# vadimkantorov/convasr

Hardware: AMD Instinct MI355X
Metric: audio-seconds/sec/node (fwd+bwd+CTC) at bs64x15s (higher is better)
Workload: dtype bf16

## Files before the change

convasr_amd/_lib.py:

```python
import ctypes
import os

import torch

_HERE = os.path.dirname(os.path.abspath(__file__))
LIB_PATH = os.environ.get('CONVASR_HIP_LIB') or os.path.join(_HERE, 'libconvasr_hip.so')

F32, BF16, I16, F16 = 0, 1, 2, 3
LOSS_SCALER_FLOATS = 8
ACT_NONE, ACT_RELU, ACT_HARDTANH, ACT_LEAKY_RELU = 0, 1, 2, 3
PACK_FWD, PACK_DGRAD = 0, 1
W_REFERENCE, W_KMAJOR = 0, 1
METRIC_CHARS, METRIC_WORDS = 0, 1
METRIC_MAX_LEN = 16383

c_int, c_i64, c_u64, c_f32, c_p = ctypes.c_int, ctypes.c_int64, ctypes.c_uint64, ctypes.c_float, ctypes.c_void_p

_SIGNATURES = dict(
	convasr_abi_version = (c_int, []),
	convasr_last_error = (ctypes.c_char_p, []),
	convasr_convert_layout = (c_int, [c_p, c_int, c_i64, c_i64, c_i64, c_p, c_int, c_i64, c_i64, c_i64, c_int, c_int, c_int, c_p]),
	convasr_signal_absmax = (c_int, [c_p, c_int, c_int, c_int, c_p, c_p]),
	convasr_logmel_fwd = (c_int, [c_p, c_int, c_p, c_p, c_p, c_int, c_p, c_p, c_p, c_int, c_int, c_int, c_int, c_int, c_f32, c_p]),
	convasr_instnorm_fwd = (c_int, [c_p, c_int, c_i64, c_i64, c_i64, c_p, c_int, c_i64, c_i64, c_i64, c_p, c_int, c_int, c_int, c_int, c_f32, c_p]),
	convasr_instnorm_running_fwd = (c_int, [c_p, c_int, c_i64, c_i64, c_i64, c_p, c_int, c_i64, c_i64, c_i64, c_int, c_int, c_int, c_int, c_f32, c_p, c_p, c_p, c_f32, c_int, c_p, c_p]),
	convasr_output_lengths = (c_int, [c_p, c_int, c_int, c_p, c_p]),
	convasr_conv_cout_pad = (c_int, [c_int]),
	convasr_pack_conv_weight = (c_int, [c_p, c_p, c_p, c_int, c_int, c_int, c_int, c_int, c_p]),
	convasr_fold2_geometry = (c_int, [c_int, c_int, ctypes.POINTER(c_int), ctypes.POINTER(c_int)]),
	convasr_fold2_pack_weight = (c_int, [c_p, c_int, c_p, c_int, c_int, c_int, c_int, c_int, c_p]),
	convasr_fold2_unfold_wgrad = (c_int, [c_p, c_p, c_int, c_int, c_int, c_int, c_int, c_int, c_p]),
	convasr_conv1d_fwd = (c_int, [c_p, c_p, c_p, c_int, c_int, c_int, c_int, c_int, c_int, c_int, c_int, c_int, c_int, c_int, c_p, c_p, c_p, c_p, c_int, c_f32, c_f32, c_p, c_p, c_p]),
	convasr_conv_stats_max_rows = (c_int, [c_int, c_int]),
	convasr_grouped_conv1d_fwd = (c_int, [c_p, c_p, c_i64, c_i64, c_i64, c_p, c_p, c_int, c_int, c_int, c_int, c_int, c_int, c_int, c_int, c_int, c_int, c_int, c_p]),
	convasr_grouped_conv1d_dgrad = (c_int, [c_p, c_p, c_p, c_i64, c_i64, c_i64, c_p, c_int, c_int, c_int, c_int, c_int, c_int, c_int, c_int, c_int, c_int, c_p]),
	convasr_grouped_conv1d_wgrad_workspace_bytes = (c_i64, [c_int, c_int, c_int, c_int, c_int]),
	convasr_grouped_conv1d_wgrad = (c_int, [c_p, c_p, c_p, c_p, c_i64, c_i64, c_i64, c_p, c_p, c_int, c_int, c_int, c_int, c_int, c_int, c_int, c_int, c_int, c_int, c_int, c_p]),
	convasr_reduce_rows = (c_int, [c_p, c_int, c_int, c_p, c_p]),
	convasr_debug_set_conv_v2 = (c_int, [c_int]),
	convasr_conv1d_wgrad_workspace_bytes = (c_i64, [c_int, c_int, c_int, c_int, c_int, c_int, c_int, c_int]),
	convasr_conv1d_wgrad = (c_int, [c_p, c_p, c_p, c_p, c_p, c_int, c_int, c_int, c_int, c_int, c_int, c_int, c_int, c_int, c_int, c_int, c_int, c_p]),
	convasr_bn_finalize = (c_int, [c_p, c_int, c_i64, c_p, c_p, c_p, c_p, c_f32, c_f32, c_p, c_p, c_p, c_p, c_int, c_p, c_p]),
	convasr_bn_eval_scale_shift = (c_int, [c_p, c_p, c_p, c_p, c_f32, c_p, c_p, c_int, c_p]),
	convasr_bn_act_fwd = (c_int, [c_p, c_p, c_int, c_p, c_p, c_int, c_p, c_p, c_p, c_int, c_f32, c_f32, c_f32, c_u64, c_u64, c_p, c_p, c_int, c_int, c_int, c_p, c_p]),
	convasr_bn_bwd_workspace_bytes = (c_i64, [c_int, c_int, c_int]),
	convasr_bn_act_bwd_reduce = (c_int, [c_p, c_p, c_p, c_int, c_p, c_p, c_p, c_p, c_int, c_p, c_p, c_p, c_p, c_p, c_p, c_int, c_f32, c_f32, c_f32, c_u64, c_u64, c_p, c_p, c_p, c_p, c_p, c_p, c_p, c_p, c_int, c_int, c_int, c_int, c_p, c_p]),
	convasr_bn_act_bwd_apply = (c_int, [c_p, c_p, c_p, c_int, c_p, c_int, c_p, c_p, c_int, c_f32, c_f32, c_f32, c_u64, c_u64, c_p, c_p, c_int, c_int, c_int, c_p, c_p]),
	convasr_bn_bwd_apply = (c_int, [c_p, c_p, c_p, c_int, c_p, c_p, c_p, c_p, c_p, c_p, c_int, c_int, c_int, c_int, c_p]),
	convasr_log_softmax_fwd = (c_int, [c_p, c_p, c_i64, c_int, c_p]),
	convasr_log_softmax_bwd = (c_int, [c_p, c_p, c_p, c_i64, c_int, c_p]),
	convasr_ctc_workspace_bytes = (c_i64, [c_int, c_int, c_int]),
	convasr_ctc_loss = (c_int, [c_p, c_p, c_p, c_p, c_p, c_p, c_p, c_int, c_int, c_int, c_int, c_int, c_p]),
	convasr_scale_rows = (c_int, [c_p, c_p, c_p, c_i64, c_p, c_int, c_i64, c_p]),
	convasr_loss_head = (c_int, [c_p, c_p, c_i64, c_p, c_int, c_f32, c_p, c_p, c_p, c_p, c_f32, c_p]),
	convasr_entropy = (c_int, [c_p, c_p, c_p, c_int, c_int, c_int, c_f32, c_p]),
	convasr_weighted_mean_entropy = (c_int, [c_p, c_p, c_p, c_int, c_int, c_int, c_int, c_f32, c_p]),
	convasr_argmax = (c_int, [c_p, c_p, c_i64, c_int, c_p]),
	convasr_sumsq_workspace_bytes = (c_i64, []),
	convasr_sumsq = (c_int, [c_p, c_i64, c_p, c_p, c_p, c_f32, c_p, c_p]),
	convasr_sgd_step = (c_int, [c_p, c_p, c_p, c_p, c_i64, c_p, c_f32, c_f32, c_f32, c_f32, c_int, c_int, c_p, c_f32, c_p, c_int, c_p, c_p, c_p, c_p]),
	convasr_adamw_step = (c_int, [c_p, c_p, c_p, c_p, c_i64, c_p, c_f32, c_f32, c_f32, c_f32, c_f32, c_f32, c_p, c_p, c_p, c_f32, c_p, c_int, c_p, c_p, c_p, c_p]),
	convasr_conv1d_dgrad_bn_reduce = (c_int, [c_p, c_p, c_p, c_int, c_int, c_int, c_int, c_int, c_int, c_int, c_int, c_int, c_p, c_p, c_p, c_p, c_p, c_int, c_f32, c_f32, c_f32, c_u64, c_u64, c_p, c_p, c_p, c_p, c_p, c_p]),
	convasr_bn_bwd_finalize = (c_int, [c_p, c_int, c_p, c_p, c_p, c_p, c_p, c_p, c_int, c_i64, c_int, c_p]),
	convasr_novograd_step = (c_int, [c_p, c_p, c_p, c_p, c_p, c_p, c_p, c_int, c_i64, c_p, c_int, c_p, c_p, c_f32, c_f32, c_f32, c_f32, c_f32, c_f32, c_int, c_int, c_p, c_p, c_f32, c_p, c_int, c_p, c_p, c_p, c_p]),
	convasr_step_begin = (c_int, [c_p, c_p]),
	convasr_conv1x1_grouped = (c_int, [c_int, c_p, c_p, c_p, c_p, c_p, c_p, c_p, c_p, c_int, c_int, c_int, ctypes.POINTER(c_int), c_p]),
	convasr_add16 = (c_int, [c_p, c_p, c_p, c_i64, c_int, c_p]),
	convasr_bn_bwd_reduce_many_workspace_bytes = (c_i64, [c_int, c_int, c_int, c_int]),
	convasr_bn_bwd_reduce_many = (c_int, [c_p, c_p, c_f32, c_p, c_int, c_p, c_p, c_p, c_p, c_p, c_p, c_p, c_p, c_p, c_int, c_int, c_int, c_int, c_p]),
	convasr_pack_dgrad_item_bytes = (c_int, []),
	convasr_pack_dgrad_grouped = (c_int, [c_p, c_int, c_int, c_p]),
	convasr_bn_finalize_grouped = (c_int, [c_int, c_p, c_int, c_i64, c_p, c_p, c_p, c_p, c_p, c_p, c_p, c_p, c_int, c_p]),
	convasr_bn_bwd_finalize_grouped = (c_int, [c_int, c_p, c_p, c_p, c_p, c_p, c_p, c_p, c_p, c_p, c_i64, c_int, c_p]),
	convasr_bn_bwd_apply_grouped = (c_int, [c_p, c_int, c_p, c_p, c_p, c_int, c_int, c_int, c_int, c_p]),
	convasr_wgrad1x1_grouped_workspace_bytes = (c_i64, [c_int, c_p, c_p, c_int, c_int]),
	convasr_wgrad1x1_grouped = (c_int, [c_int, c_p, c_p, c_p, c_p, c_p, c_p, c_p, c_p, c_int, c_int, c_int, c_p]),
	convasr_copy = (c_int, [c_p, c_p, c_i64, c_p]),
	convasr_colsum_workspace_bytes = (c_i64, [c_i64, c_int]),
	convasr_colsum = (c_int, [c_p, c_int, c_i64, c_int, c_p, c_p, c_int, c_p]),
	convasr_cast_scale = (c_int, [c_p, c_int, c_p, c_int, c_i64, c_f32, c_p]),
	convasr_bn_act_fwd_split3 = (c_int, [c_p, c_p, c_int, c_p, c_p, c_int, c_p, c_p, c_p, c_int, c_f32, c_f32, c_f32, c_u64, c_u64, c_p, c_p, c_int, c_int, c_int, c_p, c_p]),
	convasr_bn_act_bwd_apply_split3 = (c_int, [c_p, c_p, c_p, c_int, c_p, c_int, c_p, c_p, c_int, c_f32, c_f32, c_f32, c_u64, c_u64, c_p, c_p, c_int, c_int, c_int, c_p, c_p]),
	convasr_split3 = (c_int, [c_p, c_p, c_int, c_i64, c_int, c_int, c_p]),
	convasr_pack_conv_weight_split3 = (c_int, [c_p, c_int, c_p, c_p, c_int, c_int, c_int, c_int, c_int, c_p]),
	convasr_bn_act_bwd_apply_to_half = (c_int, [c_p, c_p, c_p, c_int, c_p, c_int, c_p, c_p, c_int, c_f32, c_f32, c_f32, c_u64, c_u64, c_p, c_p, c_int, c_int, c_int, c_p, c_p]),
	convasr_conv1d_fwd_splitk_plan = (c_int, [c_int, c_int, c_int, c_int, c_int, c_int, c_p]),
	convasr_conv1d_fwd_splitk = (c_int, [c_p, c_p, c_p, c_int, c_int, c_int, c_int, c_int, c_int, c_int, c_int, c_int, c_int, c_p, c_p, c_p, c_int, c_f32, c_f32, c_p, c_int, c_p, c_p]),
	convasr_conv1d_wgrad_ld_supported = (c_int, [c_int] * 10),
	convasr_conv1d_wgrad_ld = (c_int, [c_p, c_int, c_p, c_int, c_p, c_p, c_int, c_int, c_int, c_int, c_int, c_int, c_int, c_int, c_int, c_int, c_int, c_p]),
	convasr_novograd_item_elems = (c_i64, []),
	convasr_collate_pad = (c_int, [c_p, c_p, c_p, c_p, c_int, c_int, c_int, c_i64, c_p]),
	convasr_ctc_alignment_workspace_bytes = (c_i64, [c_int, c_int, c_int]),
	convasr_ctc_alignment = (c_int, [c_p, c_p, c_p, c_p, c_p, c_p, c_int, c_int, c_int, c_int, c_int, c_p]),
	convasr_ctc_alignment_long_states_per_block = (c_int, []),
	convasr_ctc_alignment_long_chunk_frames = (c_int, []),
	convasr_ctc_alignment_long_workspace_bytes = (c_i64, [c_int, c_int, c_int]),
	convasr_ctc_alignment_long = (c_int, [c_p, c_p, c_p, c_p, c_p, c_p, c_i64, c_int, c_int, c_int, c_int, c_int, c_int, c_p]),
	convasr_ctc_alignment_long_parts = (c_int, [c_p, c_p, c_p, c_p, c_p, c_p, c_i64, c_int, c_int, c_int, c_int, c_int, c_int, c_int, c_p]),
	convasr_ctc_beam_search_workspace_bytes = (c_i64, [c_int] * 6),
	convasr_ctc_beam_search = (c_int, [c_p, c_p, c_p, c_p, c_p, c_p, c_p, c_int, c_int, c_int, c_int, c_int, c_int, c_f32, c_int, c_p]),
	convasr_ctc_beam_search_lm_workspace_bytes = (c_i64, [c_int] * 6),
	convasr_ctc_beam_search_lm = (c_int, [c_p, c_p, c_p, c_p, c_p, c_p, c_p, c_int, c_int, c_int, c_int, c_int, c_int, c_f32, c_int,
	                                      c_p, c_p, c_p, c_int, c_p, c_p, c_int, c_p, c_int, c_int, c_int, c_int, ctypes.c_double, ctypes.c_double, c_p]),
	convasr_ctc_beam_search_wide_workspace_bytes = (c_i64, [c_int] * 6),
	convasr_ctc_beam_search_wide = (c_int, [c_p, c_p, c_p, c_p, c_p, c_p, c_p, c_int, c_int, c_int, c_int, c_int, c_int, c_f32, c_int, c_p]),
	convasr_ctc_beam_search_lm_wide_workspace_bytes = (c_i64, [c_int] * 6),
	convasr_ctc_beam_search_lm_wide = (c_int, [c_p, c_p, c_p, c_p, c_p, c_p, c_p, c_int, c_int, c_int, c_int, c_int, c_int, c_f32, c_int,
	                                           c_p, c_p, c_p, c_int, c_p, c_p, c_int, c_p, c_int, c_int, c_int, c_int, ctypes.c_double, ctypes.c_double, c_p]),
	convasr_edit_distance = (c_int, [c_p, c_p, c_p, c_i64, c_p, c_i64, c_p, c_p, c_int, c_int, c_int, c_int, c_int, c_i64, c_p]),
	convasr_ctc_greedy_collapse = (c_int, [c_p, c_p, c_p, c_p, c_int, c_int, c_int, c_int, c_int, c_p]),
	convasr_nw_align_workspace_bytes = (c_i64, [c_int, c_int, c_int]),
	convasr_nw_align = (c_int, [c_p, c_p, c_p, c_p, c_p, c_p, c_p, c_p, c_p, c_i64, c_int, c_int, c_int, c_int, c_int, c_int, c_int, c_p]),
	convasr_sliding_max_out_len = (c_i64, [c_i64, c_int]),
	convasr_sliding_max_tile = (c_int, [c_int]),
	convasr_sliding_max = (c_int, [c_p, c_p, c_int, c_i64, c_int, c_int, c_p]),
	convasr_kth_value_workspace_bytes = (c_i64, [c_int]),
	convasr_kth_value = (c_int, [c_p, c_p, c_p, c_i64, c_int, c_i64, c_i64, c_p]),
	convasr_scan_tile = (c_int, []),
	convasr_sign_prefix_sum_workspace_bytes = (c_i64, [c_i64]),
	convasr_sign_prefix_sum = (c_int, [c_p, c_p, c_p, c_i64, c_i64, c_p]),
	convasr_select_speaker_out_len = (c_i64, [c_i64, c_int, c_int, c_int]),
	convasr_select_speaker_workspace_bytes = (c_i64, [c_i64, c_int, c_int, c_int]),
	convasr_select_speaker = (c_int, [c_p, c_p, c_p, c_p, c_i64, c_i64, c_int, c_int, c_int, c_f32, c_f32, c_f32, c_i64, c_p]),
	convasr_rle1d_workspace_bytes = (c_i64, [c_i64]),
	convasr_rle1d_count_offset = (c_i64, [c_i64]),
	convasr_rle1d_count = (c_int, [c_p, c_int, c_int, c_i64, c_p, c_i64, c_p]),
	convasr_rle1d_write = (c_int, [c_p, c_int, c_int, c_i64, c_p, c_i64, c_i64, c_p, c_p, c_p, c_p]),
	convasr_speaker_error_counts_workspace_bytes = (c_i64, [c_i64]),
	convasr_speaker_error_counts = (c_int, [c_p, c_p, ctypes.POINTER(ctypes.c_int32), c_int, c_i64, c_p, c_p, c_i64, c_p]),
)
SLIDE_ABS, SLIDE_NEG = 1, 2
DIAR_MAX_LEN, DIAR_MAX_KERNEL, RLE_MAX_LEN, SPEAKER_MAX_PERMS = 1 << 28, 16384, 1 << 30, 8

_lib = None


class ConvasrHipError(RuntimeError):
	pass


def declared_symbols():
	return sorted(_SIGNATURES)
# ... 179 lines not shown
```

convasr_amd/csrc/conv.hip:

```cpp
#include "conv_common.h"

template <typename T, bool ALIGNED> __device__ __forceinline__ uint4 load_chunk(const T* row, int e0, int n_valid) {
	constexpr int EPC = 16 / sizeof(T);
	uint4 v = make_uint4(0, 0, 0, 0);
	if (ALIGNED) {
		if (e0 + EPC <= n_valid) v = *reinterpret_cast<const uint4*>(row + e0);
		else if (e0 < n_valid) {
			T tmp[EPC];
#pragma unroll
			for (int i = 0; i < EPC; ++i) tmp[i] = (e0 + i < n_valid) ? row[e0 + i] : (T)0;
			v = *reinterpret_cast<uint4*>(tmp);
		}
	} else if (e0 < n_valid) {
		T tmp[EPC];
#pragma unroll
		for (int i = 0; i < EPC; ++i) tmp[i] = (e0 + i < n_valid) ? row[e0 + i] : (T)0;
		v = *reinterpret_cast<uint4*>(tmp);
	}
	return v;
}

template <typename T, typename O, int XI, bool ALIGNED_X, bool SK = false>
__global__ __launch_bounds__(NTHREADS, sizeof(T) == 4 ? 1 : 2) void conv1d_igemm_kernel(ConvParams p) {
	extern __shared__ __attribute__((aligned(16))) char smem[];
// ... 639 lines not shown
#pragma unroll
				for (int tg_i = 0; tg_i < WG_TG; ++tg_i) {
					if (tg_i < ntaps) {
						uint4 bb[2];
#pragma unroll
						for (int ni = 0; ni < 2; ++ni) {
							const char* bp = xs + ((kk * 16 + kq) * p.stride + tg_i * p.dil) * PITCH + (wn * 64 + ni * 32 + colb) * 2;
							s16x4 lo = __builtin_amdgcn_ds_read_tr16_b64_v4i16((__attribute__((address_space(3))) s16x4*)(bp));
							s16x4 hi = __builtin_amdgcn_ds_read_tr16_b64_v4i16((__attribute__((address_space(3))) s16x4*)(bp + 4 * p.stride * PITCH));
							bb[ni] = make_uint4(__builtin_bit_cast(uint2, lo).x, __builtin_bit_cast(uint2, lo).y, __builtin_bit_cast(uint2, hi).x, __builtin_bit_cast(uint2, hi).y);
						}
#pragma unroll
						for (int mi = 0; mi < 2; ++mi)
#pragma unroll
							for (int ni = 0; ni < 2; ++ni) Mma<T>::run(a[mi], bb[ni], acc[tg_i][mi][ni]);
					}
				}
			}
		} else {
			const int r = lane & 31, h = lane >> 5;
#pragma unroll 4
			for (int k2 = 0; k2 < BKT / 2; ++k2) {
				float a[2];
#pragma unroll
				for (int mi = 0; mi < 2; ++mi) a[mi] = *reinterpret_cast<const float*>(ys + (k2 * 2 + h) * PITCH + (wm * 64 + mi * 32 + r) * 4);
#pragma unroll
				for (int tg_i = 0; tg_i < WG_TG; ++tg_i) {
					if (tg_i < ntaps) {
						float bb[2];
#pragma unroll
						for (int ni = 0; ni < 2; ++ni) bb[ni] = *reinterpret_cast<const float*>(xs + ((k2 * 2 + h) * p.stride + tg_i * p.dil) * PITCH + (wn * 64 + ni * 32 + r) * 4);
#pragma unroll
						for (int mi = 0; mi < 2; ++mi)
#pragma unroll
							for (int ni = 0; ni < 2; ++ni) acc[tg_i][mi][ni] = __builtin_amdgcn_mfma_f32_32x32x2f32(a[mi], bb[ni], acc[tg_i][mi][ni], 0, 0, 0);
					}
				}
			}
		}
		if (c + 1 < c_end) store_tiles(buf ^ 1);
		__syncthreads();
	}

	const int r = lane & 31, h = lane >> 5;
#pragma unroll
	for (int tg_i = 0; tg_i < WG_TG; ++tg_i) {
		if (tg_i < ntaps) {
			float* sl = p.slab + ((int64_t)split * p.K + tap0 + tg_i) * p.Cout * p.Cin;
#pragma unroll
			for (int mi = 0; mi < 2; ++mi)
#pragma unroll
				for (int ni = 0; ni < 2; ++ni) {
					const int ci = ci0 + wn * 64 + ni * 32 + r;
#pragma unroll
					for (int g = 0; g < 16; ++g) {
						const int co = co0 + wm * 64 + mi * 32 + (g & 3) + 8 * (g >> 2) + 4 * h;
						if (co < p.Cout && ci < p.Cin) sl[(int64_t)co * p.Cin + ci] = acc[tg_i][mi][ni][g];
					}
				}
		}
	}
}

__global__ __launch_bounds__(256) void wgrad_reduce_kernel(const float* __restrict__ slab, float* __restrict__ dw, int S, int K, int Cout, int Cin, int accumulate) {
	extern __shared__ float rbuf[];
	const int co = blockIdx.y, ci0 = blockIdx.x * 64;
	const int c = threadIdx.x & 63;
	const int64_t plane = (int64_t)Cout * Cin;
	for (int k = threadIdx.x >> 6; k < K; k += 4) {
		float a = 0.f;
		if (ci0 + c < Cin)
			for (int s = 0; s < S; ++s) a += slab[((int64_t)s * K + k) * plane + (int64_t)co * Cin + ci0 + c];
		rbuf[k * 65 + c] = a;
	}
	__syncthreads();
	const int ncols = min(64, Cin - ci0);
	float* out = dw + ((int64_t)co * Cin + ci0) * K;
	for (int o = threadIdx.x; o < ncols * K; o += 256) {
		const float val = rbuf[(o % K) * 65 + o / K];
		out[o] = accumulate ? out[o] + val : val;
	}
}

__global__ __launch_bounds__(256) void wgrad_reduce_kmajor_kernel(const float* __restrict__ slab, float* __restrict__ dw, int S, int64_t n4, int accumulate) {
	const float4* const s4 = reinterpret_cast<const float4*>(slab);
	float4* const d4 = reinterpret_cast<float4*>(dw);
	for (int64_t i = (int64_t)blockIdx.x * 256 + threadIdx.x; i < n4; i += (int64_t)gridDim.x * 256) {
		float4 a = s4[i];
		for (int s = 1; s < S; ++s) { const float4 b = s4[(int64_t)s * n4 + i]; a.x += b.x; a.y += b.y; a.z += b.z; a.w += b.w; }
		if (accumulate) { const float4 o = d4[i]; a.x += o.x; a.y += o.y; a.z += o.z; a.w += o.w; }
		d4[i] = a;
	}
}

template <typename T> __global__ __launch_bounds__(256) void colsum_kernel(const T* __restrict__ y, float* __restrict__ part, int64_t rows, int C, int rows_per_block) {
	__shared__ float red[4][64];
	const int c = blockIdx.x * 64 + (threadIdx.x & 63), w = threadIdx.x >> 6;
	const int64_t r0 = (int64_t)blockIdx.y * rows_per_block, r1 = min(rows, r0 + rows_per_block);
	float a = 0.f;
	if (c < C)
		for (int64_t rr = r0 + w; rr < r1; rr += 4) a += Elem<T>::load(y + rr * C + c);
	red[w][threadIdx.x & 63] = a;
	__syncthreads();
	if (w == 0 && c < C) part[(int64_t)blockIdx.y * C + c] = red[0][threadIdx.x] + red[1][threadIdx.x] + red[2][threadIdx.x] + red[3][threadIdx.x];
}
__global__ __launch_bounds__(1024) void colsum_final_kernel(const float* __restrict__ part, int nparts, int C, float* __restrict__ out, int accumulate) {
	__shared__ double red[16][64];
	const int cl = threadIdx.x & 63, c = blockIdx.x * 64 + cl, w = threadIdx.x >> 6;
	double a = 0;
	if (c < C)
		for (int i = w; i < nparts; i += 16) a += (double)part[(int64_t)i * C + c];
	red[w][cl] = a;
	__syncthreads();
	if (w != 0 || c >= C) return;
	double s = 0;
	for (int i = 0; i < 16; ++i) s += red[i][cl];
	out[c] = accumulate ? out[c] + (float)s : (float)s;
}

extern "C" int64_t convasr_colsum_workspace_bytes(int64_t rows, int C) { return ceil_div64(rows, 256) * (int64_t)C * 4; }
extern "C" int convasr_colsum(const void* y, int dtype, int64_t rows, int C, float* out, void* workspace, int accumulate, void* stream) {
	CONVASR_CHECK_ARG(y && out && workspace && rows > 0 && C > 0 && (dtype == CONVASR_F32 || convasr_is_half(dtype)), "colsum: bad arguments");
	hipStream_t s = (hipStream_t)stream;
	const int rows_per_block = 256;
	dim3 grid((C + 63) / 64, (unsigned)ceil_div64(rows, rows_per_block));
	float* part = (float*)workspace;
	if (dtype == CONVASR_F32) hipLaunchKernelGGL((colsum_kernel<float>), grid, dim3(256), 0, s, (const float*)y, part, rows, C, rows_per_block);
	else if (dtype == CONVASR_F16) hipLaunchKernelGGL((colsum_kernel<f16_t>), grid, dim3(256), 0, s, (const f16_t*)y, part, rows, C, rows_per_block);
	else hipLaunchKernelGGL((colsum_kernel<bf16_t>), grid, dim3(256), 0, s, (const bf16_t*)y, part, rows, C, rows_per_block);
	hipLaunchKernelGGL(colsum_final_kernel, dim3((C + 63) / 64), dim3(1024), 0, s, (const float*)part, (int)grid.y, C, out, accumulate);
	CONVASR_CHECK_LAUNCH("colsum");
	return 0;
}

extern "C" int64_t convasr_conv1d_wgrad_workspace_bytes(int B, int Cin, int Cout, int Tin, int Tout, int K, int stride, int dil) {
	WgradParams p;
	p.debug = 0;
	p.B = B; p.Cin = Cin; p.Cout = Cout; p.Tin = Tin; p.Tout = Tout; p.K = K; p.stride = stride; p.dil = dil;
	p.pad = 0;
	int splits = 1;
	const int bkt[3] = {64, WgTile<bf16_t>::BKT, WgTile<float>::BKT};
	const double us[3] = {1.6, 2.7, 11.0};
	for (int i = 0; i < 3; ++i) {
		WgradParams q = p;
		wgrad_plan(q, bkt[i], us[i]);
		if (q.splits > splits) splits = q.splits;
	}
	const int64_t slabs = (int64_t)splits * K * (int64_t)Cout * Cin * 4;
	const int64_t dbias_parts = ceil_div64((int64_t)B * Tout, 256) * Cout * 4;
	return slabs > dbias_parts ? slabs : dbias_parts;
}

template <typename T, int XI, bool AX, bool AY> static void launch_wgrad(const WgradParams& p, size_t smem, hipStream_t s) {
	auto kern = conv1d_wgrad_kernel<T, XI, AX, AY>;
	static unsigned long long attr_set = 0;
	convasr_allow_160k_lds(reinterpret_cast<const void*>(kern), attr_set);
	hipLaunchKernelGGL(kern, dim3(p.units * p.splits), dim3(NTHREADS), smem, s, p);
}

template <typename T> static int dispatch_wgrad(WgradParams& p, hipStream_t s) {
	wgrad_plan(p, WgTile<T>::BKT, sizeof(T) == 2 ? 2.7 : 11.0);
	const int xi = (p.x_rows * WgTile<T>::CPR + NTHREADS - 1) / NTHREADS;
	const size_t smem = 2 * (size_t)(WgTile<T>::BKT + p.x_rows) * WgTile<T>::PITCH;
	if (smem > 160 * 1024 || xi > 12) return convasr_fail(CONVASR_EUNSUPPORTED, "conv1d_wgrad: tile too large (x_rows %d)", p.x_rows);
	const bool ax = ((p.Cin * sizeof(T)) & 15) == 0, ay = ((p.Cout * sizeof(T)) & 15) == 0;
	if (ax && ay) { if (xi <= 5) launch_wgrad<T, 5, true, true>(p, smem, s); else launch_wgrad<T, 12, true, true>(p, smem, s); }
	else if (ax) launch_wgrad<T, 12, true, false>(p, smem, s);
	else if (ay) launch_wgrad<T, 12, false, true>(p, smem, s);
	else launch_wgrad<T, 12, false, false>(p, smem, s);
	return 0;
}

static int wgrad_impl(const void* x, int x_ld, const void* dy, int dy_ld, float* dw, float* dbias, void* workspace, int dtype, int B, int Cin, int Cout, int Tin,
                      int Tout, int K, int stride, int dil, int pad, int accumulate, int dw_layout, void* stream) {
	CONVASR_CHECK_ARG(x && dy && dw && workspace && B > 0 && Cin > 0 && Cout > 0 && Tin > 0 && Tout > 0 && K > 0 && stride > 0 && dil > 0 && (dw_layout == CONVASR_W_REFERENCE || dw_layout == CONVASR_W_KMAJOR), "conv1d_wgrad: bad arguments");
	CONVASR_CHECK_ARG(dw_layout == CONVASR_W_REFERENCE || (((int64_t)Cout * Cin) & 3) == 0, "conv1d_wgrad: K-major dw needs Cout * Cin %% 4 == 0");
	CONVASR_CHECK_ARG(K <= 64, "conv1d_wgrad: K %d > 64", K);
	WgradParams p;
	p.debug = g_conv_debug;
	p.x = x; p.dy = dy; p.slab = (float*)workspace;
	p.B = B; p.Cin = Cin; p.Cout = Cout; p.Tin = Tin; p.Tout = Tout; p.K = K; p.stride = stride; p.dil = dil; p.pad = pad;
	p.x_ld = x_ld == Cin ? 0 : x_ld; p.dy_ld = dy_ld == Cout ? 0 : dy_ld;
	hipStream_t s = (hipStream_t)stream;
	int rc;
	if (convasr_is_half(dtype) && g_conv_use_v2 && convasr_wgrad_v2_try(p, dtype, s)) rc = 0;
	else if (p.x_ld || p.dy_ld) return convasr_fail(CONVASR_EUNSUPPORTED, "conv1d_wgrad_ld: frames %d / %d elements apart need the LDS-DMA kernel's envelope (16-bit storage, stride 1, Cin %% 128 == 0, Cout %% 128 == 0)", x_ld, dy_ld);
	else if (dtype == CONVASR_F32) rc = dispatch_wgrad<float>(p, s);
	else if (dtype == CONVASR_BF16) rc = dispatch_wgrad<bf16_t>(p, s);
	else if (dtype == CONVASR_F16) rc = dispatch_wgrad<f16_t>(p, s);
	else return convasr_fail(CONVASR_EUNSUPPORTED, "conv1d_wgrad: dtype %d", dtype);
	if (rc) return rc;
	CONVASR_CHECK_LAUNCH("conv1d_wgrad");
	if (dw_layout == CONVASR_W_KMAJOR) {
		const int64_t n4 = (int64_t)K * Cout * Cin / 4;
		int64_t blocks = ceil_div64(n4, 256);
		if (blocks > 2048) blocks = 2048;
		hipLaunchKernelGGL(wgrad_reduce_kmajor_kernel, dim3((unsigned)blocks), dim3(256), 0, s, (const float*)p.slab, dw, p.splits, n4, accumulate);
	} else hipLaunchKernelGGL(wgrad_reduce_kernel, dim3((Cin + 63) / 64, Cout), dim3(256), (size_t)K * 65 * sizeof(float), s, p.slab, dw, p.splits, K, Cout, Cin, accumulate);
	CONVASR_CHECK_LAUNCH("conv1d_wgrad_reduce");
	if (dbias) {
		const int64_t rows = (int64_t)B * Tout;
		const int rows_per_block = 256;
		dim3 grid((Cout + 63) / 64, (unsigned)ceil_div64(rows, rows_per_block));
		float* part = p.slab;
		if (dtype == CONVASR_F32) hipLaunchKernelGGL((colsum_kernel<float>), grid, dim3(256), 0, s, (const float*)dy, part, rows, Cout, rows_per_block);
		else if (dtype == CONVASR_F16) hipLaunchKernelGGL((colsum_kernel<f16_t>), grid, dim3(256), 0, s, (const f16_t*)dy, part, rows, Cout, rows_per_block);
		else hipLaunchKernelGGL((colsum_kernel<bf16_t>), grid, dim3(256), 0, s, (const bf16_t*)dy, part, rows, Cout, rows_per_block);
		hipLaunchKernelGGL(colsum_final_kernel, dim3((Cout + 63) / 64), dim3(1024), 0, s, (const float*)part, (int)grid.y, Cout, dbias, accumulate);
		CONVASR_CHECK_LAUNCH("conv1d_dbias");
	}
	return 0;
}

extern "C" int convasr_conv1d_wgrad(const void* x, const void* dy, float* dw, float* dbias, void* workspace, int dtype, int B, int Cin, int Cout, int Tin,
                                    int Tout, int K, int stride, int dil, int pad, int accumulate, int dw_layout, void* stream) {
	return wgrad_impl(x, 0, dy, 0, dw, dbias, workspace, dtype, B, Cin, Cout, Tin, Tout, K, stride, dil, pad, accumulate, dw_layout, stream);
}

extern "C" int convasr_conv1d_wgrad_ld(const void* x, int x_ld, const void* dy, int dy_ld, float* dw, void* workspace, int dtype, int B, int Cin, int Cout, int Tin,
                                       int Tout, int K, int dil, int pad, int accumulate, int dw_layout, void* stream) {
	CONVASR_CHECK_ARG(x_ld >= Cin && dy_ld >= Cout && (x_ld & 7) == 0 && (dy_ld & 7) == 0 && convasr_is_half(dtype), "conv1d_wgrad_ld: x_ld >= Cin, dy_ld >= Cout, multiples of 8, 16-bit storage");
	return wgrad_impl(x, x_ld, dy, dy_ld, dw, nullptr, workspace, dtype, B, Cin, Cout, Tin, Tout, K, 1, dil, pad, accumulate, dw_layout, stream);
}

extern "C" int convasr_conv1d_wgrad_ld_supported(int dtype, int B, int Cin, int Cout, int Tin, int Tout, int K, int dil, int x_ld, int dy_ld) {
	if (!convasr_is_half(dtype) || B <= 0 || Cin <= 0 || Cout <= 0 || Tin <= 0 || Tout <= 0 || K <= 0 || K > 64 || dil <= 0 || x_ld < Cin || dy_ld < Cout) return 0;
	WgradParams p = WgradParams();
	p.B = B; p.Cin = Cin; p.Cout = Cout; p.Tin = Tin; p.Tout = Tout; p.K = K; p.stride = 1; p.dil = dil;
	p.x_ld = x_ld == Cin ? 0 : x_ld; p.dy_ld = dy_ld == Cout ? 0 : dy_ld;
	return g_conv_use_v2 && convasr_wgrad_v2_supports(p);
}

static bool fold2_geometry(int K, int pad, int* Kf, int* Pf, int* s0) {
	if (K < 1 || pad < 0) return false;
	*Pf = (pad + 1) / 2;
	*s0 = 2 * *Pf - pad;
	*Kf = (K - 1 + *s0) / 2 + 1;
	return true;
}

extern "C" int convasr_fold2_geometry(int K, int pad, int* K_folded, int* pad_folded) {
	int s0;
	CONVASR_CHECK_ARG(K_folded && pad_folded && fold2_geometry(K, pad, K_folded, pad_folded, &s0), "fold2_geometry: bad arguments");
	return 0;
}

template <typename T>
__global__ __launch_bounds__(256) void fold2_pack_kernel(const float* __restrict__ w, int kmajor, T* __restrict__ wf, int Cout, int CoutPad, int Cin, int K, int Kf, int s0) {
	const int64_t n = (int64_t)Kf * CoutPad * 2 * Cin;
	for (int64_t i = (int64_t)blockIdx.x * 256 + threadIdx.x; i < n; i += (int64_t)gridDim.x * 256) {
		const int c2 = (int)(i % (2 * Cin));
		const int64_t r = i / (2 * Cin);
		const int co = (int)(r % CoutPad), j = (int)(r / CoutPad);
		const int p = c2 >= Cin ? 1 : 0, ci = c2 - p * Cin, k = 2 * j + p - s0;
		float v = 0.f;
		if (co < Cout && k >= 0 && k < K) v = kmajor ? w[((int64_t)k * Cout + co) * Cin + ci] : w[((int64_t)co * Cin + ci) * K + k];
		Elem<T>::store(wf + i, v);
	}
}

extern "C" int convasr_fold2_pack_weight(const float* w, int w_layout, void* packed_fwd, int dtype, int Cout, int Cin, int K, int pad, void* stream) {
	int Kf, Pf, s0;
	CONVASR_CHECK_ARG(w && packed_fwd && Cout > 0 && Cin > 0 && fold2_geometry(K, pad, &Kf, &Pf, &s0) && (w_layout == CONVASR_W_REFERENCE || w_layout == CONVASR_W_KMAJOR), "fold2_pack_weight: bad arguments");
	const int co_pad = convasr_conv_cout_pad(Cout);
	int64_t blocks = ceil_div64((int64_t)Kf * co_pad * 2 * Cin, 256);
	if (blocks > 2048) blocks = 2048;
	if (dtype == CONVASR_BF16) hipLaunchKernelGGL((fold2_pack_kernel<bf16_t>), dim3((unsigned)blocks), dim3(256), 0, (hipStream_t)stream, w, w_layout == CONVASR_W_KMAJOR, (bf16_t*)packed_fwd, Cout, co_pad, Cin, K, Kf, s0);
	else if (dtype == CONVASR_F16) hipLaunchKernelGGL((fold2_pack_kernel<f16_t>), dim3((unsigned)blocks), dim3(256), 0, (hipStream_t)stream, w, w_layout == CONVASR_W_KMAJOR, (f16_t*)packed_fwd, Cout, co_pad, Cin, K, Kf, s0);
	else if (dtype == CONVASR_F32) hipLaunchKernelGGL((fold2_pack_kernel<float>), dim3((unsigned)blocks), dim3(256), 0, (hipStream_t)stream, w, w_layout == CONVASR_W_KMAJOR, (float*)packed_fwd, Cout, co_pad, Cin, K, Kf, s0);
	else return convasr_fail(CONVASR_EUNSUPPORTED, "fold2_pack_weight: dtype %d", dtype);
	CONVASR_CHECK_LAUNCH("fold2_pack_weight");
	return 0;
}

__global__ __launch_bounds__(256) void fold2_unfold_kernel(const float* __restrict__ dwf, float* __restrict__ dw, int kmajor, int Cout, int Cin, int K, int s0, int accumulate) {
	const int64_t n = (int64_t)K * Cout * Cin;
	for (int64_t i = (int64_t)blockIdx.x * 256 + threadIdx.x; i < n; i += (int64_t)gridDim.x * 256) {
		int k, co, ci;
		if (kmajor) { ci = (int)(i % Cin); const int64_t r = i / Cin; co = (int)(r % Cout); k = (int)(r / Cout); }
		else { k = (int)(i % K); const int64_t r = i / K; ci = (int)(r % Cin); co = (int)(r / Cin); }
		const int j = (k + s0) >> 1, p = (k + s0) & 1;
		const float v = dwf[((int64_t)j * Cout + co) * 2 * Cin + p * Cin + ci];
		dw[i] = accumulate ? dw[i] + v : v;
	}
}

extern "C" int convasr_fold2_unfold_wgrad(const float* dw_folded, float* dw, int dw_layout, int Cout, int Cin, int K, int pad, int accumulate, void* stream) {
	int Kf, Pf, s0;
	CONVASR_CHECK_ARG(dw_folded && dw && Cout > 0 && Cin > 0 && fold2_geometry(K, pad, &Kf, &Pf, &s0) && (dw_layout == CONVASR_W_REFERENCE || dw_layout == CONVASR_W_KMAJOR), "fold2_unfold_wgrad: bad arguments");
	int64_t blocks = ceil_div64((int64_t)K * Cout * Cin, 256);
	if (blocks > 2048) blocks = 2048;
	hipLaunchKernelGGL(fold2_unfold_kernel, dim3((unsigned)blocks), dim3(256), 0, (hipStream_t)stream, dw_folded, dw, dw_layout == CONVASR_W_KMAJOR, Cout, Cin, K, s0, accumulate);
	CONVASR_CHECK_LAUNCH("fold2_unfold_wgrad");
	return 0;
}
```

convasr_amd/csrc/misc.hip:

```cpp
#include "common.h"

thread_local char g_convasr_err[512] = {0};

int convasr_fail(int code, const char* fmt, ...) {
	va_list ap;
	va_start(ap, fmt);
	vsnprintf(g_convasr_err, sizeof(g_convasr_err), fmt, ap);
	va_end(ap);
	return code;
}

extern "C" int convasr_abi_version(void) { return CONVASR_ABI_VERSION; }
extern "C" const char* convasr_last_error(void) { return g_convasr_err; }

template <typename S, typename D>
__global__ __launch_bounds__(256) void convert_layout_kernel(const S* __restrict__ src, int64_t ssb, int64_t ssc, int64_t sst,
                                                             D* __restrict__ dst, int64_t dsb, int64_t dsc, int64_t dst_st, int C, int T) {
	__shared__ float tile[64][65];
	const int b = blockIdx.z, c0 = blockIdx.y * 64, t0 = blockIdx.x * 64;
	const int tx = threadIdx.x & 63, ty = threadIdx.x >> 6;
	const bool src_t_fast = (sst == 1) || (ssc != 1), dst_t_fast = (dst_st == 1) || (dsc != 1);
#pragma unroll 4
	for (int i = 0; i < 16; ++i) {
		int c = src_t_fast ? c0 + ty + 4 * i : c0 + tx, t = src_t_fast ? t0 + tx : t0 + ty + 4 * i;
// ... 339 lines not shown
}

extern "C" int convasr_cast_scale(const void* src, int src_dtype, void* dst, int dst_dtype, int64_t n, float scale, void* stream) {
	CONVASR_CHECK_ARG(src && dst && n > 0 && (n & 7) == 0 && ((src_dtype == CONVASR_F32 && convasr_is_half(dst_dtype)) || (convasr_is_half(src_dtype) && dst_dtype == CONVASR_F32)), "cast_scale: n %% 8 == 0, fp32 -> bf16 / fp16 or back");
	int64_t blocks = ceil_div64(n >> 3, 256);
	if (blocks > 8192) blocks = 8192;
	const dim3 g((unsigned)blocks), b(256);
	hipStream_t s = (hipStream_t)stream;
	if (src_dtype == CONVASR_F32) CONVASR_DISPATCH_HALF(dst_dtype, H, hipLaunchKernelGGL((cast_scale_kernel<float, H>), g, b, 0, s, (const float*)src, (H*)dst, n >> 3, scale));
	else CONVASR_DISPATCH_HALF(src_dtype, H, hipLaunchKernelGGL((cast_scale_kernel<H, float>), g, b, 0, s, (const H*)src, (float*)dst, n >> 3, scale));
	CONVASR_CHECK_LAUNCH("cast_scale");
	return 0;
}

__global__ __launch_bounds__(256) void copy_kernel(const unsigned char* __restrict__ src, unsigned char* __restrict__ dst, int64_t n16, int64_t nbytes, int aligned) {
	const int64_t i0 = (int64_t)blockIdx.x * 256 + threadIdx.x, step = (int64_t)gridDim.x * 256;
	if (aligned) {
		for (int64_t i = i0; i < n16; i += step) reinterpret_cast<uint4*>(dst)[i] = reinterpret_cast<const uint4*>(src)[i];
		for (int64_t i = n16 * 16 + i0; i < nbytes; i += step) dst[i] = src[i];
	} else {
		for (int64_t i = i0; i < nbytes; i += step) dst[i] = src[i];
	}
}

extern "C" int convasr_copy(const void* src, void* dst, int64_t nbytes, void* stream) {
	CONVASR_CHECK_ARG(src && dst && nbytes >= 0, "copy: bad arguments");
	if (nbytes == 0) return 0;
	const int aligned = ((((uintptr_t)src) | ((uintptr_t)dst)) & 15) == 0;
	const int64_t n16 = aligned ? nbytes >> 4 : 0;
	int64_t blocks = ceil_div64(aligned ? (n16 > 0 ? n16 : 1) : nbytes, 256);
	if (blocks > 4096) blocks = 4096;
	hipLaunchKernelGGL(copy_kernel, dim3((unsigned)blocks), dim3(256), 0, (hipStream_t)stream, (const unsigned char*)src, (unsigned char*)dst, n16, nbytes, aligned);
	CONVASR_CHECK_LAUNCH("copy");
	return 0;
}

extern "C" int convasr_loss_head(const float* loss_vec, const int64_t* ylen, int64_t ylen_stride, const float* entropy, int B, float accumulate_iterations, float* out3,
                                 float* grad_loss_vec, unsigned char* skipped, const float* loss_scaler, float metric_scale, void* stream) {
	CONVASR_CHECK_ARG(loss_vec && ylen && out3 && B > 0 && accumulate_iterations > 0.f, "loss_head: bad arguments");
	hipLaunchKernelGGL(loss_head_kernel, dim3(1), dim3(256), 0, (hipStream_t)stream, loss_vec, ylen, ylen_stride, entropy, B, accumulate_iterations, out3, grad_loss_vec, skipped, loss_scaler, metric_scale);
	CONVASR_CHECK_LAUNCH("loss_head");
	return 0;
}

#define SUMSQ_BLOCKS 2048
__global__ __launch_bounds__(256) void sumsq_kernel(const float* __restrict__ g, int64_t n, double* __restrict__ part) {
	__shared__ float red[4];
	float acc = 0.f;
	const int64_t n4 = n >> 2;
	const float4* g4 = reinterpret_cast<const float4*>(g);
	for (int64_t i = (int64_t)blockIdx.x * 256 + threadIdx.x; i < n4; i += (int64_t)gridDim.x * 256) {
		float4 v = g4[i];
		acc += v.x * v.x + v.y * v.y + v.z * v.z + v.w * v.w;
	}
	if (blockIdx.x == 0 && threadIdx.x < (n & 3)) { float v = g[n4 * 4 + threadIdx.x]; acc += v * v; }
	acc = wave_sum(acc);
	if ((threadIdx.x & 63) == 0) red[threadIdx.x >> 6] = acc;
	__syncthreads();
	if (threadIdx.x == 0) part[blockIdx.x] = (double)red[0] + (double)red[1] + (double)red[2] + (double)red[3];
}

__global__ __launch_bounds__(256) void sumsq_final_kernel(const double* __restrict__ part, int blocks, double* __restrict__ out, float* __restrict__ norm_out, float norm_scale, const float* __restrict__ scaler) {
	__shared__ double red[256];
	double a = 0;
	for (int i = threadIdx.x; i < blocks; i += 256) a += part[i];
	red[threadIdx.x] = a;
	__syncthreads();
	if (threadIdx.x == 0) { double s = 0; for (int i = 0; i < 256; ++i) s += red[i]; *out = s; if (norm_out) *norm_out = (float)(sqrt(s) * (double)norm_scale) * (scaler ? 1.f / scaler[LS_SCALE] : 1.f); }
}

extern "C" int64_t convasr_sumsq_workspace_bytes(void) { return SUMSQ_BLOCKS * (int64_t)sizeof(double); }

extern "C" int convasr_sumsq(const float* g, int64_t n, double* sumsq, void* workspace, float* norm_out, float norm_scale, const float* loss_scaler, void* stream) {
	CONVASR_CHECK_ARG(g && sumsq && workspace && n > 0, "sumsq: bad arguments");
	CONVASR_CHECK_ARG(((uintptr_t)g & 15) == 0, "sumsq: g must be 16-byte aligned");
	int64_t blocks = ceil_div64(n, 1024);
	if (blocks > SUMSQ_BLOCKS) blocks = SUMSQ_BLOCKS;
	hipLaunchKernelGGL(sumsq_kernel, dim3((unsigned)blocks), dim3(256), 0, (hipStream_t)stream, g, n, (double*)workspace);
	hipLaunchKernelGGL(sumsq_final_kernel, dim3(1), dim3(256), 0, (hipStream_t)stream, (const double*)workspace, (int)blocks, sumsq, norm_out, norm_scale, loss_scaler);
	CONVASR_CHECK_LAUNCH("sumsq");
	return 0;
}

template <typename H> __global__ __launch_bounds__(256) void sgd_step_kernel(float* __restrict__ p, const float* __restrict__ g, float* __restrict__ buf, float* __restrict__ gout,
                                                       int64_t n, const double* __restrict__ sumsq, float max_norm, float lr, float mom, float wd, int nesterov, int first,
                                                       const float* __restrict__ loss_gate, float grad_scale, H* __restrict__ p16, const float* __restrict__ scaler_in, float* __restrict__ scaler_out, const float* __restrict__ lr_dev) {
	if (lr_dev) lr = *lr_dev;
	const bool gated = loss_gate && !(fabsf(*loss_gate) < INFINITY);
	const LossScale ls = loss_scale_read(scaler_in, (scaler_in && sumsq) ? *sumsq : 0.0);
	if (scaler_in && blockIdx.x == 0 && threadIdx.x == 0) loss_scale_advance(scaler_in, scaler_out, ls.overflow, gated);
	if (gated || ls.overflow) return;
	grad_scale *= ls.inv;
	float clip = 1.f;
	if (sumsq && max_norm > 0.f) {
		float total = (float)sqrt(*sumsq) * grad_scale;
		float c = max_norm / (total + 1e-6f);
		clip = c < 1.f ? c : 1.f;
	}
	clip *= grad_scale;
	auto update = [&](float gi, float pv, float& bv, float& gout_v) {
		const float gc = gi * clip;
		gout_v = gc;
		float d = gc + wd * pv;
		if (mom != 0.f) {
			bv = first ? d : mom * bv + d;
			d = nesterov ? d + mom * bv : bv;
		}
		return pv - lr * d;
	};
	const int64_t n4 = n >> 2;
	for (int64_t i = (int64_t)blockIdx.x * 256 + threadIdx.x; i < n4; i += (int64_t)gridDim.x * 256) {
		const float4 g4 = reinterpret_cast<const float4*>(g)[i], p4 = reinterpret_cast<const float4*>(p)[i];
		float4 b4 = make_float4(0.f, 0.f, 0.f, 0.f), o4;
		if (mom != 0.f && !first) b4 = reinterpret_cast<const float4*>(buf)[i];
		float4 r;
		r.x = update(g4.x, p4.x, b4.x, o4.x); r.y = update(g4.y, p4.y, b4.y, o4.y); r.z = update(g4.z, p4.z, b4.z, o4.z); r.w = update(g4.w, p4.w, b4.w, o4.w);
		reinterpret_cast<float4*>(p)[i] = r;
		if (mom != 0.f) reinterpret_cast<float4*>(buf)[i] = b4;
		if (gout) reinterpret_cast<float4*>(gout)[i] = o4;
		if (p16) reinterpret_cast<uint2*>(p16)[i] = make_uint2(pack16<H>(r.x, r.y), pack16<H>(r.z, r.w));
	}
	if (blockIdx.x == 0 && (int64_t)threadIdx.x < (n & 3)) {
		const int64_t i = (n4 << 2) + threadIdx.x;
		float bv = (mom != 0.f && !first) ? buf[i] : 0.f, go;
		const float r = update(g[i], p[i], bv, go);
		p[i] = r;
		if (mom != 0.f) buf[i] = bv;
		if (gout) gout[i] = go;
		if (p16) Elem<H>::store(p16 + i, r);
	}
}

extern "C" int convasr_sgd_step(float* p, const float* g, float* buf, float* grad_out, int64_t n, const double* sumsq, float max_norm, float lr,
                                float momentum, float weight_decay, int nesterov, int first, const float* loss_gate, float grad_scale, void* p16, int p16_dtype,
                                const float* scaler_in, float* scaler_out, const float* lr_dev, void* stream) {
	CONVASR_CHECK_ARG(p && g && n > 0 && (momentum == 0.f || buf), "sgd_step: bad arguments");
	CONVASR_CHECK_ARG(!p16 || convasr_is_half(p16_dtype), "sgd_step: the mirror's dtype must be CONVASR_BF16 or CONVASR_F16");
	CONVASR_CHECK_ARG((scaler_in == nullptr) == (scaler_out == nullptr) && (!scaler_in || (scaler_in != scaler_out && sumsq)), "sgd_step: the loss scaler needs distinct in / out states and the gradient's sum of squares (its overflow check)");
	int64_t blocks = ceil_div64(n, 256);
	if (blocks > 4096) blocks = 4096;
	CONVASR_DISPATCH_HALF(p16_dtype, H, hipLaunchKernelGGL((sgd_step_kernel<H>), dim3((unsigned)blocks), dim3(256), 0, (hipStream_t)stream, p, g, buf, grad_out, n, sumsq, max_norm, lr, momentum, weight_decay, nesterov, first, loss_gate, grad_scale, (H*)p16, scaler_in, scaler_out, lr_dev));
	CONVASR_CHECK_LAUNCH("sgd_step");
	return 0;
}

template <typename H> __global__ __launch_bounds__(256) void adamw_step_kernel(float* __restrict__ p, const float* __restrict__ g, float* __restrict__ m, float* __restrict__ v,
                                                         int64_t n, const double* __restrict__ sumsq, float max_norm, float lr, float beta1, float beta2, float eps, float wd,
                                                         const float* __restrict__ step_in, float* __restrict__ step_out, const float* __restrict__ loss_gate, float grad_scale,
                                                         H* __restrict__ p16, const float* __restrict__ scaler_in, float* __restrict__ scaler_out, const float* __restrict__ lr_dev) {
	if (lr_dev) lr = *lr_dev;
	const bool gated = loss_gate && !(fabsf(*loss_gate) < INFINITY);
	const LossScale ls = loss_scale_read(scaler_in, (scaler_in && sumsq) ? *sumsq : 0.0);
	const float t0 = *step_in;
	if (blockIdx.x == 0 && threadIdx.x == 0) {
		if (scaler_in) loss_scale_advance(scaler_in, scaler_out, ls.overflow, gated);
		*step_out = (gated || ls.overflow) ? t0 : t0 + 1.f;
	}
	if (gated || ls.overflow) return;
	grad_scale *= ls.inv;
	float clip = 1.f;
	if (sumsq && max_norm > 0.f) {
		const float total = (float)sqrt(*sumsq) * grad_scale;
		const float c = max_norm / (total + 1e-6f);
		clip = c < 1.f ? c : 1.f;
	}
	clip *= grad_scale;
// ... 42 lines not shown
```

convasr_amd/functional.py:

```python
import os

import torch

from . import ops, _lib

_pack_cache = {}
_param_epoch = [0]


def bump_param_epoch():
	_param_epoch[0] += 1


def param_version(w):
	return (w._version, w.data_ptr(), _param_epoch[0])


def packed_weight(w, dtype, mode):
	ver = param_version(w)
	ent = _pack_cache.get((id(w), dtype))
	if ent is not None:
		if mode == _lib.PACK_DGRAD:
			if ent['dgr_ver'] == ver:
				return ent['dgr']
# ... 15 lines not shown
			ent['fwd_ver'] = ver if flat._mirror_ver.get(id(w)) == ver else None
			ent['flat'], ent['mirror'] = flat, flat.data16
	if mode == _lib.PACK_FWD and ent['fwd_ver'] == ver:
		return ent['fwd']
	if mode == _lib.PACK_DGRAD and ent['dgr_ver'] == ver:
		return ent['dgr']
	if mode == _lib.PACK_DGRAD:
		ent['fwd'], ent['dgr'] = ops.pack_weight(w, dtype, None, out = (ent['fwd'], ent['dgr']), fwd_is_current = ent['fwd_ver'] == ver)
		ent['fwd_ver'] = ent['dgr_ver'] = ver
	else:
		ent['fwd'] = ops.pack_weight(w, dtype, _lib.PACK_FWD, out = (ent['fwd'], None))
		ent['fwd_ver'] = ver
	if in_place and dtype in ops.HALF_DTYPES:
		arena[0]._mirror_ver[id(w)] = ver
	return ent['fwd'] if mode == _lib.PACK_FWD else ent['dgr']


_structure_epoch = [0]


def invalidate_pack_cache():
	_pack_cache.clear()
	_split_cache.clear()
	_structure_epoch[0] += 1


_split_cache = {}


def force_repack():
	for ent in _pack_cache.values():
		ent['dgr_ver'] = None
		if ent.get('flat') is None:
			ent['fwd_ver'] = None
	for cache in (Fold2._cache, _HeadPad._cache, _split_cache):
		for ent in cache.values():
			ent['ver'] = None


def split_weight(w, dtype, dgrad_planes = 3):
	ver = param_version(w)
	ent = _split_cache.get((id(w), dtype, dgrad_planes))
	if ent is None:
		ent = _split_cache[(id(w), dtype, dgrad_planes)] = dict(w = w, ver = None, fwd = None, dgr = None)
	if ent['ver'] != ver:
		ent['fwd'], ent['dgr'] = ops.pack_weight_split3(w, dtype, out = (ent['fwd'], ent['dgr']), dgrad_planes = dgrad_planes)
		ent['ver'] = ver
	return ent['fwd'], ent['dgr']


_PLANES_ATTR = '_convasr_planes_only'
_PLANES_CACHE_ATTR = '_convasr_planes_cache'
_nan_cells = {}


def _planes_placeholder(z3, B, C, T):
	dev = z3.device
	cell = _nan_cells.get(dev)
	if cell is None:
		cell = _nan_cells[dev] = torch.full((1, ), float('nan'), dtype = torch.float32, device = dev)
	z = cell.as_strided((B, C, T), (0, 0, 0))
	setattr(z, _PLANES_ATTR, z3)
	return z


def _take_planes(x):
	d = getattr(x, '__dict__', None)
	return d.pop(_PLANES_ATTR, None) if d else None


def split_applies(split, dt, spec, Cin, Cout):
	return split is not None and dt == torch.float32 and spec.stride == 1 and Cin % 64 == 0 and Cout % 8 == 0


def structure_epoch():
	return _structure_epoch[0]


PREPACK = os.environ.get('CONVASR_NO_PREPACK') != '1'
GRAPHS_CAPTURED = [False]
_prepack_streams = {}


GROUPED_PACK_MIN = int(os.environ.get('CONVASR_GROUPED_PACK_MIN', 32))
_pack_tables = {}


def _pack_group(stale, dtype, refresh = True):
	group = []
	if dtype in ops.HALF_DTYPES and len(stale) >= GROUPED_PACK_MIN:
		for w in stale:
			ent = _pack_cache.get((id(w), dtype))
			if ent is None or ent['dgr'] is None:
				continue
			fwd = packed_weight(w, dtype, _lib.PACK_FWD) if refresh else ent['fwd']
			Cout, Cin, K = w.shape
			if fwd is not None and Cout % 2 == 0 and Cin % 2 == 0 and fwd.dtype == dtype:
				group.append((w, ent, fwd))
	return group


def _pack_table(group, dtype):
	import struct
	dev = group[0][0].device
	key = tuple((fwd.data_ptr(), ent['dgr'].data_ptr()) for _, ent, fwd in group)
	tab = _pack_tables.get((dev, dtype, key))
	if tab is None:
		if capturing():
			raise _lib.ConvasrHipError('the dgrad pack table changed while a step graph is being captured (GraphedTrainStep prewarms it: functional.prewarm_dgrad_pack)')
		assert _lib.load().convasr_pack_dgrad_item_bytes() == 40
		blob, first = b'', 0
		for w, ent, fwd in group:
			Cout, Cin, K = w.shape
			blob += struct.pack('<QQiiiiii', fwd.data_ptr(), ent['dgr'].data_ptr(), Cout, Cin, K, ops.cout_pad(Cout), ops.cout_pad(Cin), first)
			first += K * ((Cout + 63) // 64) * ((Cin + 63) // 64)
		tab = _pack_tables[(dev, dtype, key)] = dict(key = key, items = torch.frombuffer(bytearray(blob), dtype = torch.uint8).to(dev), blocks = first, n = len(group))
	return tab


def prewarm_dgrad_pack(weights, dtype):
	group = _pack_group([w for w in weights], dtype, refresh = False)
	if group:
		_pack_table(group, dtype)


def _pack_dgrad_many(stale, dtype):
	group = _pack_group(stale, dtype)
	grouped = {id(w) for w, _, _ in group}
	for w in stale:
		if id(w) not in grouped:
			packed_weight(w, dtype, _lib.PACK_DGRAD)
	if not group:
		return
	tab = _pack_table(group, dtype)
	_lib.call('convasr_pack_dgrad_grouped', _lib.ptr(tab['items']), tab['n'], tab['blocks'], _lib.stream_ptr())
	for w, ent, _ in group:
		ent['dgr_ver'] = param_version(w)


def prepack_dgrad_weights(weights, dtype):
	if not weights:
		return
	dev = weights[0].device
	join_prepack(dev)
	stale = []
	for w in weights:
		ent = _pack_cache.get((id(w), dtype))
		if ent is None or ent['dgr'] is None:
			packed_weight(w, dtype, _lib.PACK_DGRAD)
		elif ent['dgr_ver'] != param_version(w):
			stale.append(w)
	if not stale:
		return
	if not PREPACK or GRAPHS_CAPTURED[0]:
		_pack_dgrad_many(stale, dtype)
		return
	st = _prepack_streams.get(dev)
	if st is None:
		st = _prepack_streams[dev] = [torch.cuda.Stream(device = dev), False]
	side, main = st[0], torch.cuda.current_stream(dev)
	_lib.stream_wait(side, main)
	with torch.cuda.stream(side):
		_pack_dgrad_many(stale, dtype)
	st[1] = True


def join_prepack(device):
	st = _prepack_streams.get(device)
	if st is not None and st[1]:
		_lib.stream_wait(torch.cuda.current_stream(device), st[0])
		st[1] = False


CAPTURING = ops._capturing


def capturing():
	return CAPTURING[0]


class _DropoutState:
	seed = 0x5EEDC0DE
	offset = 0
	dev = {}

	@classmethod
	def next(cls, numel):
		off = cls.offset
		cls.offset += (numel + 3) // 4 + 1
		return cls.seed, off

	@classmethod
	def key(cls, device):
		st = cls.dev.get(device)
		return None if st is None else st['state'].data_ptr() + 16

	@classmethod
	def upload(cls, device):
		signed = cls.seed - (1 << 64) if cls.seed >= (1 << 63) else cls.seed
		st = cls.dev.get(device)
		if st is None:
			st = cls.dev[device] = dict(state = torch.zeros(4, dtype = torch.int64, device = device), seed = None)
		st['state'].copy_(torch.tensor([signed, 0, 0, 0], dtype = torch.int64))
		st['seed'] = cls.seed
		return st


def manual_seed(seed):
	_DropoutState.seed = int(seed) & 0xFFFFFFFFFFFFFFFF
	_DropoutState.offset = 0
	for device in list(_DropoutState.dev):
		_DropoutState.upload(device)


def begin_step(device):
	device = torch.device(device)
	st = _DropoutState.dev.get(device)
	if st is None or st['seed'] != _DropoutState.seed:
		if CAPTURING[0]:
			raise _lib.ConvasrHipError('begin_step: the dropout state of this device must exist before a step is captured (run one eager step first)')
		st = _DropoutState.upload(device)
	_lib.call('convasr_step_begin', st['state'].data_ptr(), _lib.stream_ptr())
	_DropoutState.offset = 0


def _deliver(params, compute):
	live = [p is not None and p.requires_grad for p in params]
	if not any(live):
		return [None] * len(params)
	arenas = [getattr(p, '_convasr_grad', None) if ok else None for p, ok in zip(params, live)]
	if all(a is not None for a, ok in zip(arenas, live) if ok):
		fresh = {bool(getattr(p, '_convasr_fresh', True)) for p, ok in zip(params, live) if ok}
		if len(fresh) != 1:
			raise _lib.ConvasrHipError('gradient arenas of one layer are out of step (mixed fresh / accumulated state)')
		compute(arenas, not fresh.pop())
		for p, ok in zip(params, live):
			if ok:
				p._convasr_fresh = False
				hook = getattr(p, '_convasr_ready', None)
				if hook is not None:
					hook(p)
		return [None] * len(params)
	outs = [torch.empty_like(p, dtype = torch.float32, memory_format = torch.contiguous_format) if ok else None for p, ok in zip(params, live)]
	compute(outs, False)
	return outs


def _deliver_many(groups, compute):
	outs, accs, ret, arena_groups = [], [], [], []
	for params in groups:
		live = [p is not None and p.requires_grad for p in params]
		arenas = [getattr(p, '_convasr_grad', None) if ok else None for p, ok in zip(params, live)]
		if any(live) and all(a is not None for a, ok in zip(arenas, live) if ok):
			fresh = {bool(getattr(p, '_convasr_fresh', True)) for p, ok in zip(params, live) if ok}
			if len(fresh) != 1:
				raise _lib.ConvasrHipError('gradient arenas of one layer are out of step (mixed fresh / accumulated state)')
			outs.append(arenas); accs.append(not fresh.pop()); ret.append([None] * len(params)); arena_groups.append((params, live))
		else:
			o = [torch.empty_like(p, dtype = torch.float32, memory_format = torch.contiguous_format) if ok else None for p, ok in zip(params, live)]
			outs.append(o); accs.append(False); ret.append(o)
	compute(outs, accs)
	for params, live in arena_groups:
		for p, ok in zip(params, live):
			if ok:
				p._convasr_fresh = False
				hook = getattr(p, '_convasr_ready', None)
				if hook is not None:
					hook(p)
	return ret


GROUP_RES = os.environ.get('CONVASR_NO_GROUPED_RES') != '1'
_GACC_ATTR = '_convasr_gacc'
RES_WGRAD_SIDE = os.environ.get('CONVASR_NO_RES_WGRAD_SIDE') != '1'
after_long_launch_hooks = {}
_side_streams = {}


def enable_side_stream_wgrad(device, enabled = True):
	device = torch.device(device)
	_side_streams[device] = torch.cuda.Stream(device = device) if enabled else None


def side_stream(device):
	return _side_streams.get(torch.device(device))


SIDE_KEEPALIVE = os.environ.get('CONVASR_NO_SIDE_KEEPALIVE') != '1'
_side_keepalive = {}


def join_side_streams():
	for dev, side in _side_streams.items():
		if side is not None:
			_lib.stream_wait(torch.cuda.current_stream(dev), side)
	_wgrad_pending.clear()
	for held in _side_keepalive.values():
		del held[:]


WGRAD_AFTER_DGRAD = os.environ.get('CONVASR_WGRAD_AFTER_DGRAD', '0') == '1'
_wgrad_pending = {}


def _join_pending_wgrad(dev):
	if _wgrad_pending.pop(dev, False):
		side = _side_streams.get(dev)
		if side is not None:
			torch.cuda.current_stream(dev).wait_stream(side)


def _run_wgrad(dev, tensors, fn):
	side = _side_streams.get(dev)
	if side is None:
		return fn()
	if WGRAD_AFTER_DGRAD:
		_wgrad_pending[dev] = True
	_lib.stream_wait(side, torch.cuda.current_stream(dev))
	with torch.cuda.stream(side):
		out = fn()
	held = _side_keepalive.setdefault(dev, [])
	if SIDE_KEEPALIVE and len(held) < 16384:
		held.extend(tensors)
	else:
		for t in tensors:
			t.record_stream(side)
	return out


SPLIT_FAMILY, SPLIT_WGRAD_FAMILY = 'conv1d_igemm_v2s_kernel<x3>', 'conv1d_wgrad<x3>'


class ConvSpec:

	def __init__(self, K, stride = 1, dilation = 1, padding = 0):
		self.K, self.stride, self.dilation, self.padding = K, stride, dilation, padding


class Fold2:
	_cache = {}
# ... 260 lines not shown
			dz = ops.add16(dz, acc, out = acc)
		link, fused_sums = ctx.bwd_link, None
		if link is not None:
			if link['dz'] is not None and link['dz'].data_ptr() == dz.data_ptr() and link['dz'].shape == dz.shape:
				fused_sums = link['sums']
			link['dz'] = None

		if n_res == 0 and fused_sums is not None:
			coef = torch.empty(3 * Cout, dtype = torch.float32, device = dev)
			finalize = lambda outs, acc: ops.bn_bwd_finalize(fused_sums, gamma, bnp[0], bnp[1], B * Tout, coef = coef, dgamma = outs[0], dbeta = outs[1], accumulate = acc)
			if gamma.requires_grad or beta.requires_grad:
				dgamma, dbeta = _deliver([gamma, beta], finalize)
			else:
				finalize([None, None], False)
				dgamma = dbeta = None
			dy = ops.bn_act_bwd_apply(dz, y, coef, True, bnp[2], bnp[3], act, xlen = xl, dropout_p = p_drop, seed = seed, offset = offset, gate = ctx.gate, step_key = skey, planes = ctx.split, hi_only = hi)
			g = rsum_of = None
		elif n_res == 0:
			coef = torch.empty(3 * Cout, dtype = torch.float32, device = dev)
			reduce = lambda outs, acc: ops.bn_act_bwd_reduce(dz, y, bnp[2], bnp[3], bnp[0], bnp[1], act, xlen = xl, dropout_p = p_drop, seed = seed, offset = offset, write_g = False, gamma = gamma, coef = coef, dgamma = outs[0], dbeta = outs[1], accumulate = acc, gate = ctx.gate, step_key = skey)
			if gamma.requires_grad or beta.requires_grad:
				dgamma, dbeta = _deliver([gamma, beta], reduce)
			else:
				reduce([None, None], False)
				dgamma = dbeta = None
			dy = ops.bn_act_bwd_apply(dz, y, coef, True, bnp[2], bnp[3], act, xlen = xl, dropout_p = p_drop, seed = seed, offset = offset, gate = ctx.gate, step_key = skey, planes = ctx.split, hi_only = hi)
			g = rsum_of = None
		else:
			bn_idx = [r for r in range(n_res) if res_bnp[r] is not None]
			grouped_bn = None
			if ctx.gate is not None and GROUP_RES and dt in ops.HALF_DTYPES and 1 + len(bn_idx) <= 13:
				sets = [(gamma, beta, bnp, y)] + [(ctx.params[3 + 4 * r + 2], ctx.params[3 + 4 * r + 3], res_bnp[r], res_y[r]) for r in bn_idx]
				coefs = torch.empty(len(sets), 3 * Cout, dtype = torch.float32, device = dev)
				holder = {}
				def many(outs, accs):
					holder['g'] = ops.bn_bwd_reduce_many(dz, ctx.gate, p_drop, [t[3] for t in sets], [t[2][0] for t in sets], [t[2][1] for t in sets], [t[0] for t in sets], [coefs[i] for i in range(len(sets))], [o[0] for o in outs], [o[1] for o in outs], accs)
				dgb = _deliver_many([[gm, bt] for gm, bt, _, _ in sets], many)
				g = holder['g']
				dys = ops.bn_bwd_apply_grouped(g, [t[3] for t in sets], [coefs[i] for i in range(len(sets))])
				(dgamma, dbeta), dy = dgb[0], dys[0]
				grouped_bn = {r: (dgb[1 + i][0], dgb[1 + i][1], dys[1 + i]) for i, r in enumerate(bn_idx)}
				rsum_of = None
		if n_res > 0 and grouped_bn is None:
			sums = torch.empty(2 * Cout * (1 + len(bn_idx)), dtype = torch.float64, device = dev)
			rsum_of = {r: sums[2 * Cout * (1 + i):2 * Cout * (2 + i)] for i, r in enumerate(bn_idx)}
			common = dict(xlen = xl, res = res_y, rscale = [None if p is None else p[2] for p in res_bnp], rshift = [None if p is None else p[3] for p in res_bnp], rmean = [None if p is None else p[0] for p in res_bnp], rinvstd = [None if p is None else p[1] for p in res_bnp], dropout_p = p_drop, seed = seed, offset = offset, step_key = skey)
			first = [r for r in bn_idx if r < 2]
			g = ops.bn_act_bwd_reduce(dz, y, bnp[2], bnp[3], bnp[0], bnp[1], act, rsums = [rsum_of.get(r) if r in first else None for r in range(n_res)], sums = sums[:2 * Cout], **common)
			rest = [r for r in bn_idx if r >= 2]
			while rest:
				batch, rest = rest[:2], rest[2:]
				ops.bn_act_bwd_reduce(g, g, None, None, None, None, (_lib.ACT_NONE, 0.0, 0.0), res = [res_y[r] for r in batch], rscale = [None] * len(batch), rshift = [None] * len(batch), rmean = [common['rmean'][r] for r in batch], rinvstd = [common['rinvstd'][r] for r in batch], rsums = [rsum_of[r] for r in batch], write_g = False)
			grouped_bn = GROUP_RES and dt in ops.HALF_DTYPES and len(bn_idx) >= 1 and len(bn_idx) <= 12
			if grouped_bn:
				coefs = torch.empty(1 + len(bn_idx), 3 * Cout, dtype = torch.float32, device = dev)
				sets = [(gamma, beta, bnp, sums[:2 * Cout])] + [(ctx.params[3 + 4 * r + 2], ctx.params[3 + 4 * r + 3], res_bnp[r], rsum_of[r]) for r in bn_idx]
				dgb = _deliver_many([[gm, bt] for gm, bt, _, _ in sets], lambda outs, accs: ops.bn_bwd_finalize_grouped([t[3] for t in sets], [t[0] for t in sets], [t[2][0] for t in sets], [t[2][1] for t in sets], B * Tout,
					[coefs[i] for i in range(len(sets))], [o[0] for o in outs], [o[1] for o in outs], accs))
				dys = ops.bn_bwd_apply_grouped(g, [y] + [res_y[r] for r in bn_idx], [coefs[i] for i in range(len(sets))])
				(dgamma, dbeta), dy = dgb[0], dys[0]
				grouped_bn = {r: (dgb[1 + i][0], dgb[1 + i][1], dys[1 + i]) for i, r in enumerate(bn_idx)}
			else:
				dgamma, dbeta, dy = _bn_backward_from_g(g, y, gamma, beta, bnp, sums[:2 * Cout], B * Tout)

		if n_res == 0:
			grouped_bn = None
		arena_mode = getattr(weight, '_convasr_grad', None) is not None
		if ctx.split is not None and dy.dtype == torch.float32:
			dy = ops.as_cl(dy, ctx.split) if hi else ops.split3(dy, ctx.split, ops.SPLIT_GRAD)
		if hi and ctx.fold is not None:
			wg = lambda: _deliver([weight], lambda outs, acc: Fold2.wgrad_hi(x, dy, weight, spec, ctx.fold[0], ctx.fold[1], outs[0], acc))
		elif hi:
			wg = lambda: _deliver([weight], lambda outs, acc: ops.conv1d_wgrad_hi(x, dy, Cout, spec.K, spec.dilation, spec.padding, outs[0], accumulate = acc))
		elif ctx.split is not None and ctx.fold is not None:
			wg = lambda: _deliver([weight], lambda outs, acc: Fold2.wgrad_split(x, dy, weight, spec, ctx.fold[0], ctx.fold[1], outs[0], acc))
		elif ctx.split is not None:
			xf, dyf = ops.split3_frames(x), ops.split3_frames(dy)
			wg = lambda: _deliver([weight], lambda outs, acc: ops.conv1d_wgrad(xf, dyf, Cout, spec.K, 1, 3 * spec.dilation, 3 * spec.padding, outs[0], accumulate = acc, work = 2.0 * B * Tout * Cout * weight.shape[1] * spec.K, family = SPLIT_WGRAD_FAMILY))
		elif ctx.fold is not None:
			Bx, Cin, Tin = x.shape
			xv = x.as_strided((Bx, 2 * Cin, Tin // 2), (Tin * Cin, 1, 2 * Cin))
			wg = lambda: _deliver([weight], lambda outs, acc: Fold2.wgrad(xv, dy, weight, spec, ctx.fold[0], ctx.fold[1], outs[0], acc))
		else:
			wg = lambda: _deliver([weight], lambda outs, acc: ops.conv1d_wgrad(x, dy, Cout, spec.K, spec.stride, spec.dilation, spec.padding, outs[0], accumulate = acc))
		after = WGRAD_AFTER_DGRAD and arena_mode and _side_streams.get(dev) is not None
		if arena_mode and not after:
			dw, = _run_wgrad(dev, (x, dy), wg)
		dx = None
		if ctx.x_needs_grad:
			if spec.stride != 1:
				raise _lib.ConvasrHipError('conv1d dgrad with stride > 1 is not implemented (only the prologue conv is strided and its input needs no gradient)')
			dx = _dgrad(x, dy, weight, spec, dt, ctx.producer_link, split = ctx.split, hi = hi)
		if after:
			dw, = _run_wgrad(dev, (x, dy), wg)
		if not arena_mode:
			dw, = wg()

		res_grads = [None] * (5 * n_res)
		pending = []
		wg_group = []
		for r in range(n_res):
			rw, rb, rg, rbeta = ctx.params[3 + 4 * r:3 + 4 * r + 4]
			rx = res_x[r]
			need_rx = ctx.needs_input_grad[6 + 5 * r]
			if res_bnp[r] is None:
				res_grads[5 * r] = g if need_rx else None
				continue
			p = res_bnp[r]
			drg, drbeta, dry = grouped_bn[r] if grouped_bn else _bn_backward_from_g(g, res_y[r], rg, rbeta, p, rsum_of[r], B * Tout)
			drx = None
			if ctx.res_split[r]:
				sp, cin_r = cfg['split'], rw.shape[1]
				hi_r = bool(cfg.get('split_hi_bwd'))
				dry3 = ops.as_cl(dry, sp) if hi_r else ops.split3(dry, sp, ops.SPLIT_GRAD)
				if need_rx and hi_r:
					drx = ops.conv1d(dry3, split_weight(rw, sp, 1)[1], cin_r, 1, 1, 1, 0, out_dtype = torch.float32)
				elif need_rx:
					drx = ops.conv1d(dry3, split_weight(rw, sp)[1], cin_r, 1, 1, 1, 0, out_dtype = torch.float32, work = 2.0 * B * Tout * Cout * cin_r, family = SPLIT_FAMILY)

				def res_wgrad3(outs, acc, rx3 = rx, dry3 = dry3, rb = rb, cin_r = cin_r, hi_r = hi_r):
					if hi_r:
						ops.conv1d_wgrad_hi(rx3, dry3, Cout, 1, 1, 0, outs[0], accumulate = acc)
					else:
						ops.conv1d_wgrad(ops.split3_frames(rx3), ops.split3_frames(dry3), Cout, 1, 1, 3, 0, outs[0], accumulate = acc, work = 2.0 * B * Tout * Cout * cin_r, family = SPLIT_WGRAD_FAMILY)
					if outs[1] is not None and not acc and not (outs[1] is getattr(rb, '_convasr_grad', None) and getattr(rb, '_convasr_grad_is_zero', False)):
						outs[1].zero_()
						rb._convasr_grad_is_zero = outs[1] is getattr(rb, '_convasr_grad', None)
				drw, drb = _deliver([rw, rb], res_wgrad3)
				res_grads[5 * r:5 * r + 5] = [drx, drw, drb, drg, drbeta]
				continue
			if need_rx and ctx.res_gacc[r] is not None and rx.shape[1] % 128 == 0 and Cout % 64 == 0:
				pending.append((r, dry))
			elif need_rx:
				join_prepack(dry.device)
				drx = ops.conv1d(dry, packed_weight(rw, dt, _lib.PACK_DGRAD), rx.shape[1], 1, 1, 1, 0)
			arena = getattr(rw, '_convasr_grad', None) is not None and (rb is None or getattr(rb, '_convasr_grad', None) is not None)
			if GROUP_RES and arena and rw.requires_grad and dt in ops.HALF_DTYPES and rx.shape[1] % 128 == 0 and Cout % 128 == 0 and (rb is None or rb.requires_grad):
				wg_group.append((r, rx, dry))
				res_grads[5 * r:5 * r + 5] = [drx, None, None, drg, drbeta]
				continue
			def res_wgrad(outs, acc, rx = rx, dry = dry, rb = rb):
				ops.conv1d_wgrad(rx, dry, Cout, 1, 1, 1, 0, outs[0], accumulate = acc)
				if outs[1] is not None and not acc and not (outs[1] is getattr(rb, '_convasr_grad', None) and getattr(rb, '_convasr_grad_is_zero', False)):
					outs[1].zero_()
					rb._convasr_grad_is_zero = outs[1] is getattr(rb, '_convasr_grad', None)
			if RES_WGRAD_SIDE and arena:
				drw, drb = _run_wgrad(dry.device, (rx, dry), lambda rw = rw, rb = rb, f = res_wgrad: _deliver([rw, rb], f))
			else:
				drw, drb = _deliver([rw, rb], res_wgrad)
			res_grads[5 * r:5 * r + 5] = [drx, drw, drb, drg, drbeta]
		if pending:
			join_prepack(dev)
			accs = [ctx.res_gacc[r] for r, _ in pending]
			fresh = [a['buf'] is None for a in accs]
			for (r, _), a, fr in zip(pending, accs, fresh):
				if fr:
					a['buf'] = ops.empty_cl(B, res_x[r].shape[1], Tout, dt, dev)
			done = ops.conv1x1_grouped([dry for _, dry in pending], [packed_weight(ctx.params[3 + 4 * r], dt, _lib.PACK_DGRAD) for r, _ in pending], [res_x[r].shape[1] for r, _ in pending], outs = [a['buf'] for a in accs], accumulate = [not fr for fr in fresh])
			if done is None:
				raise _lib.ConvasrHipError('grouped input gradient of the residual branches: a shape left the one-tap kernel\'s envelope between forward and backward')
		if wg_group:
			ps = [(ctx.params[3 + 4 * r], ctx.params[3 + 4 * r + 1]) for r, _, _ in wg_group]
			fresh = [bool(getattr(w, '_convasr_fresh', True)) for w, _ in ps]
			if any(b is not None and bool(getattr(b, '_convasr_fresh', True)) != fr for (_, b), fr in zip(ps, fresh)):
				raise _lib.ConvasrHipError('gradient arenas of one residual branch are out of step (mixed fresh / accumulated state)')

			def run():
# ... 85 lines not shown

class ConvBiasFunction(torch.autograd.Function):

	@staticmethod
	def forward(ctx, cfg, x, weight, bias):
		spec, dt = cfg['spec'], cfg['compute_dtype']
		ctx.producer_link = _take_link(x)
		x = ops.as_cl(x, dt)
		Cout, Cin, K = weight.shape
		ctx.split = None
		if cfg.get('split') is not None and dt == torch.float32 and K == 1 and spec.stride == 1 and spec.padding == 0 and Cin % 128 == 0 and Cout <= HEAD_PAD and os.environ.get('CONVASR_NO_HEAD_PAD') != '1':
			ctx.split = cfg['split']
			B, _, T = x.shape
			x = ops.split3(x, ctx.split, ops.SPLIT_INPUT)
			y = ops.conv1d(x, _HeadPad.split_weight(weight, ctx.split, 1 if cfg.get('split_hi_bwd') else 3)[0], Cout, 1, 1, 1, 0, out_dtype = cfg.get('out_dtype', torch.float32), bias = bias, work = 2.0 * B * T * Cout * Cin, family = SPLIT_FAMILY)
		else:
			y = ops.conv1d(x, packed_weight(weight, dt, _lib.PACK_FWD), weight.shape[0], spec.K, spec.stride, spec.dilation, spec.padding, out_dtype = cfg.get('out_dtype', torch.float32), bias = bias)
		ctx.cfg = cfg
		ctx.params = (weight, bias)
		ctx.save_for_backward(x)
		return y

	@staticmethod
	def backward(ctx, dy):
		cfg = ctx.cfg
		spec, dt = cfg['spec'], cfg['compute_dtype']
		weight, bias = ctx.params
		x, = ctx.saved_tensors
		Cout = weight.shape[0]
		if ctx.split is not None:
			Cin = weight.shape[1]
			B, _, T = dy.shape
			dy = ops.as_cl(dy, torch.float32)
			hi = bool(cfg.get('split_hi_bwd'))
			dy3 = _HeadPad.pad_grad(dy, ctx.split) if hi else ops.split3(_HeadPad.pad_grad(dy, torch.float32), ctx.split, ops.SPLIT_GRAD)
			dx = None
			if ctx.needs_input_grad[1] and hi:
				dx = ops.conv1d(dy3, _HeadPad.split_weight(weight, ctx.split, 1)[1], Cin, 1, 1, 1, 0, out_dtype = torch.float32, work = 2.0 * B * T * Cout * Cin)
				_after_long_launch()
			elif ctx.needs_input_grad[1]:
				dx = ops.conv1d(dy3, _HeadPad.split_weight(weight, ctx.split)[1], Cin, 1, 1, 1, 0, out_dtype = torch.float32, work = 2.0 * B * T * Cout * Cin, family = SPLIT_FAMILY)
				_after_long_launch()

			def wgrad3(outs, acc):
				dwp = torch.empty(HEAD_PAD, Cin, 1, dtype = torch.float32, device = dy.device)
				if hi:
					ops.conv1d_wgrad_hi(x, dy3, HEAD_PAD, 1, 1, 0, dwp, work = 2.0 * B * T * Cout * Cin)
				else:
					ops.conv1d_wgrad(ops.split3_frames(x), ops.split3_frames(dy3), HEAD_PAD, 1, 1, 3, 0, dwp, work = 2.0 * B * T * Cout * Cin, family = SPLIT_WGRAD_FAMILY)
				if outs[0] is not None:
					v = dwp[:Cout]
					if acc:
						outs[0].add_(v.view(outs[0].shape))
					else:
						_lib.call('convasr_convert_layout', _lib.ptr(v), _lib.F32, 0, v.stride(0), v.stride(1), _lib.ptr(outs[0]), _lib.F32, 0, outs[0].stride(0), outs[0].stride(1), 1, Cout, Cin, _lib.stream_ptr())
				if outs[1] is not None:
					ops.colsum(dy, outs[1], accumulate = acc)
			dw, db = _deliver([weight, bias], wgrad3)
			return None, dx, dw, db
		if dt in ops.HALF_DTYPES and spec.K == 1 and spec.stride == 1 and spec.padding == 0 and Cout < HEAD_PAD and x.shape[1] % 128 == 0 and os.environ.get('CONVASR_NO_HEAD_PAD') != '1':
			dyp = _HeadPad.pad_grad(dy, dt)
			dx = _dgrad(x, dyp, weight, spec, dt, ctx.producer_link, wd = _HeadPad.dgrad_weight(weight, dt)) if ctx.needs_input_grad[1] else None

			def wgrad(outs, acc):
				dwp = torch.empty(HEAD_PAD, x.shape[1], 1, dtype = torch.float32, device = x.device)
				dbp = torch.empty(HEAD_PAD, dtype = torch.float32, device = x.device) if outs[1] is not None else None
				ops.conv1d_wgrad(x, dyp, HEAD_PAD, 1, 1, 1, 0, dwp, dbias = dbp)
				for o, v in ((outs[0], dwp[:Cout]), (outs[1], None if dbp is None else dbp[:Cout].view(Cout, 1, 1))):
					if o is None:
						continue
					if acc:
						o.add_(v.view(o.shape))
					else:
						ov = o.view(Cout, -1, 1) if o.ndim == 1 else o
						_lib.call('convasr_convert_layout', _lib.ptr(v), _lib.F32, 0, v.stride(0), v.stride(1), _lib.ptr(ov), _lib.F32, 0, ov.stride(0), ov.stride(1), 1, Cout, v.shape[1], _lib.stream_ptr())
			dw, db = _deliver([weight, bias], wgrad)
			return None, dx, dw, db
		dy = ops.as_cl(dy, dt)
		dx = None
		if ctx.needs_input_grad[1]:
			if spec.stride != 1:
				raise _lib.ConvasrHipError('conv1d dgrad with stride > 1 is not implemented')
			dx = _dgrad(x, dy, weight, spec, dt, ctx.producer_link)
		dw, db = _deliver([weight, bias], lambda outs, acc: ops.conv1d_wgrad(x, dy, Cout, spec.K, spec.stride, spec.dilation, spec.padding, outs[0], dbias = outs[1], accumulate = acc))
		return None, dx, dw, db


class GroupedConvReluFunction(torch.autograd.Function):

	@staticmethod
	def forward(ctx, cfg, x, weight, bias):
		spec, dt = cfg['spec'], cfg['compute_dtype']
		_take_link(x)
		x = ops.as_cl(x, dt)
		y = ops.grouped_conv1d(x, weight.detach(), None if bias is None else bias.detach(), cfg['groups'], spec.stride, spec.padding, relu = True)
		ctx.cfg, ctx.params = cfg, (weight, bias)
		ctx.save_for_backward(x, y)
		return y

	@staticmethod
	def backward(ctx, dy):
		cfg = ctx.cfg
		spec, dt, groups = cfg['spec'], cfg['compute_dtype'], cfg['groups']
		weight, bias = ctx.params
		x, y = ctx.saved_tensors
		dy = ops.as_cl(dy, dt)
		dx = ops.grouped_conv1d_dgrad(dy, y, weight.detach(), x.shape[1], x.shape[2], groups, spec.stride, spec.padding) if ctx.needs_input_grad[1] else None
		dw, db = _deliver([weight, bias], lambda outs, acc: ops.grouped_conv1d_wgrad(x, dy, y, outs[0], outs[1], groups, spec.stride, spec.padding, accumulate = acc))
		return None, dx, dw, db


class ConvBnActEvalFunction:

	@staticmethod
	def apply(cfg, x, weight, bias, scale_shift, xlen, res_list):
		spec, dt, act = cfg['spec'], cfg['compute_dtype'], cfg['act']
		x = ops.as_cl(x, dt)
		Cout = weight.shape[0]
		xl = ops.xlen_f32(xlen, x.device) if (cfg['temporal_mask'] and xlen is not None) else None
		scale, shift = (None, None) if scale_shift is None else (scale_shift[0], scale_shift[1])
		fold = Fold2.plan(x, weight, spec, dt, False)
		sk = not torch.is_grad_enabled()
		split = cfg.get('split_eval')
		if fold is not None:
			xv, Kf, Pf, Tout = fold
			conv = lambda **epilogue: ops.conv1d(xv, Fold2.packed_weight(weight, dt, spec.padding), Cout, Kf, 1, 1, Pf, bias = bias, Tout = Tout, work = 2.0 * x.shape[0] * Tout * Cout * x.shape[1] * spec.K, splitk = sk, **epilogue)
		elif split_applies(split, dt, spec, x.shape[1], Cout):
			x3, wp3 = ops.split3(x, split, ops.SPLIT_INPUT), split_weight(weight, split)[0]
			conv = lambda **epilogue: ops.conv1d(x3, wp3, Cout, spec.K, 1, spec.dilation, spec.padding, out_dtype = torch.float32, bias = bias, work = 2.0 * x.shape[0] * ops.conv_out_len(x.shape[2], spec.K, 1, spec.dilation, spec.padding) * Cout * x.shape[1] * spec.K, family = SPLIT_FAMILY, splitk = sk, **epilogue)
		else:
			wp = packed_weight(weight, dt, _lib.PACK_FWD)
			conv = lambda **epilogue: ops.conv1d(x, wp, Cout, spec.K, spec.stride, spec.dilation, spec.padding, bias = bias, splitk = sk, **epilogue)
		p_drop = float(cfg.get('dropout_p', 0.0))
		if not res_list and p_drop == 0:
			return conv(scale = scale, shift = shift, act = act, xlen = xl)
		y = conv()
		res_y, rscale, rshift = [], [], []
		for rx, rw, rb, rss in res_list:
			rx = ops.as_cl(rx, dt)
			if rw is None:
				res_y.append(rx); rscale.append(None); rshift.append(None)
			elif split_applies(split, dt, ConvSpec(1), rx.shape[1], Cout):
				res_y.append(ops.conv1d(ops.split3(rx, split, ops.SPLIT_INPUT), split_weight(rw, split)[0], Cout, 1, 1, 1, 0, out_dtype = torch.float32, bias = rb, work = 2.0 * rx.shape[0] * rx.shape[2] * Cout * rx.shape[1], family = SPLIT_FAMILY, splitk = sk))
				rscale.append(None if rss is None else rss[0]); rshift.append(None if rss is None else rss[1])
			else:
				res_y.append(ops.conv1d(rx, packed_weight(rw, dt, _lib.PACK_FWD), Cout, 1, 1, 1, 0, bias = rb, splitk = sk))
				rscale.append(None if rss is None else rss[0]); rshift.append(None if rss is None else rss[1])
		seed, offset = _DropoutState.next(y.numel()) if p_drop > 0 else (0, 0)
		return ops.bn_act(y, scale, shift, act, xlen = xl, res = res_y, rscale = rscale, rshift = rshift, dropout_p = p_drop, seed = seed, offset = offset, step_key = _DropoutState.key(y.device) if p_drop > 0 else None)


class ConvBnActFrozenStatsFunction(torch.autograd.Function):

	@staticmethod
	def _affine(bn, gamma, beta):
		if bn is None or not isinstance(bn, torch.nn.modules.batchnorm._BatchNorm):
			return None, None, None, None
		ss = ops.bn_eval_scale_shift(gamma, beta, bn.running_mean, bn.running_var, bn.eps)
		return ss[0], ss[1], bn.running_mean.detach().float(), torch.rsqrt(bn.running_var.detach().float() + bn.eps)

	@staticmethod
	def forward(ctx, cfg, x, weight, bias, gamma, beta, xlen, *flat_res):
		spec, dt, act = cfg['spec'], cfg['compute_dtype'], cfg['act']
		ctx.producer_link = _take_link(x)
		x = ops.as_cl(x, dt)
		dev = x.device
		Cout = weight.shape[0]
		xl = ops.xlen_f32(xlen, dev) if (cfg['temporal_mask'] and xlen is not None) else None
		y = ops.conv1d(x, packed_weight(weight, dt, _lib.PACK_FWD), Cout, spec.K, spec.stride, spec.dilation, spec.padding, bias = bias)
		aff = ConvBnActFrozenStatsFunction._affine(cfg['bn'], gamma, beta)
		n_res = len(flat_res) // 5
		res_x, res_y, res_aff = [], [], []
		for r in range(n_res):
			rx, rw, rb, rg, rbeta = flat_res[5 * r:5 * r + 5]
			rx = ops.as_cl(rx, dt)
			res_x.append(rx)
			if rw is None:
				res_y.append(rx); res_aff.append((None, None, None, None))
			else:
				res_y.append(ops.conv1d(rx, packed_weight(rw, dt, _lib.PACK_FWD), Cout, 1, 1, 1, 0, bias = rb))
				res_aff.append(ConvBnActFrozenStatsFunction._affine(cfg['res_bn'][r], rg, rbeta))
		p_drop = cfg['dropout_p']
		seed, offset = _DropoutState.next(y.numel()) if p_drop > 0 else (0, 0)
		skey = _DropoutState.key(dev) if p_drop > 0 else None
		z = ops.bn_act(y, aff[0], aff[1], act, xlen = xl, res = res_y, rscale = [a[0] for a in res_aff], rshift = [a[1] for a in res_aff], dropout_p = p_drop, seed = seed, offset = offset, step_key = skey)
		ctx.cfg, ctx.n_res, ctx.drop = cfg, n_res, (p_drop, seed, offset, skey)
		ctx.params = (weight, bias, gamma, beta) + tuple(flat_res[5 * r + k] for r in range(n_res) for k in range(1, 5))
		ctx.aff, ctx.res_aff = aff, res_aff
		ctx.x_needs_grad = x.requires_grad or ctx.needs_input_grad[1]
		ctx.save_for_backward(x, y, xl, *res_x, *res_y)
		return z

	@staticmethod
	def _coef(scale, C, dev):
		coef = torch.zeros(3 * C, dtype = torch.float32, device = dev)
		coef[:C] = 1.0 if scale is None else scale
		return coef

	@staticmethod
	def backward(ctx, dz):
		cfg, n_res = ctx.cfg, ctx.n_res
		spec, dt, act = cfg['spec'], cfg['compute_dtype'], cfg['act']
		saved = ctx.saved_tensors
		x, y, xl = saved[:3]
		res_x, res_y = list(saved[3:3 + n_res]), list(saved[3 + n_res:3 + 2 * n_res])
		weight, bias, gamma, beta = ctx.params[:4]
		scale, shift, rmean, rinv = ctx.aff
		p_drop, seed, offset, skey = ctx.drop
		B, Cout, Tout = y.shape
		dev = y.device
		dz = ops.as_cl(dz, dt)
		live = lambda p: p is not None and p.requires_grad
		common = dict(xlen = xl, res = res_y, rscale = [a[0] for a in ctx.res_aff], rshift = [a[1] for a in ctx.res_aff], dropout_p = p_drop, seed = seed, offset = offset, step_key = skey)
		dgamma = dbeta = None
		if scale is not None and (live(gamma) or live(beta)):
			sums = torch.empty(2 * Cout, dtype = torch.float64, device = dev)
			scratch = torch.empty(3 * Cout, dtype = torch.float32, device = dev)
			holder = {}
			def reduce(outs, acc):
				holder['g'] = ops.bn_act_bwd_reduce(dz, y, scale, shift, rmean, rinv, act, sums = sums, write_g = True, gamma = gamma, coef = scratch, dgamma = outs[0], dbeta = outs[1], accumulate = acc, **common)
			dgamma, dbeta = _deliver([gamma, beta], reduce)
			g = holder['g']
		else:
			g = ops.bn_act_bwd_reduce(dz, y, scale, shift, None, None, act, write_g = True, **common)
		dy = g if scale is None else ops.bn_act_bwd_apply(g, y, ConvBnActFrozenStatsFunction._coef(scale, Cout, dev), False)
		dw, db = _deliver([weight, bias], lambda outs, acc: ops.conv1d_wgrad(x, dy, Cout, spec.K, spec.stride, spec.dilation, spec.padding, outs[0], dbias = outs[1], accumulate = acc))
		dx = None
		if ctx.x_needs_grad:
			if spec.stride != 1:
				raise _lib.ConvasrHipError('conv1d dgrad with stride > 1 is not implemented (only the prologue conv is strided and its input needs no gradient)')
			dx = _dgrad(x, dy, weight, spec, dt, ctx.producer_link)
		res_grads = []
		for r in range(n_res):
			rw, rb, rg, rbeta = ctx.params[4 + 4 * r:4 + 4 * r + 4]
			need_rx = ctx.needs_input_grad[7 + 5 * r]
			if rw is None:
				res_grads += [g if need_rx else None, None, None, None, None]
				continue
			rscale, rshift, rrm, rri = ctx.res_aff[r]
			drg = drbeta = None
			if rscale is not None and (live(rg) or live(rbeta)):
				rs = torch.empty(2 * Cout, dtype = torch.float64, device = dev)
				ops.bn_act_bwd_reduce(g, g, None, None, None, None, (_lib.ACT_NONE, 0.0, 0.0), res = [res_y[r]], rscale = [None], rshift = [None], rmean = [rrm], rinvstd = [rri], rsums = [rs], write_g = False)
				def put(outs, acc, rs = rs):
					for o, v in ((outs[0], rs[Cout:]), (outs[1], rs[:Cout])):
						if o is not None:
							o.add_(v.float()) if acc else o.copy_(v.float())
				drg, drbeta = _deliver([rg, rbeta], put)
			dry = g if rscale is None else ops.bn_act_bwd_apply(g, res_y[r], ConvBnActFrozenStatsFunction._coef(rscale, Cout, dev), False)
			join_prepack(dev)
			drx = ops.conv1d(dry, packed_weight(rw, dt, _lib.PACK_DGRAD), res_x[r].shape[1], 1, 1, 1, 0) if need_rx else None
			if rb is not None:
				rb._convasr_grad_is_zero = False
			drw, drb = _deliver([rw, rb], lambda outs, acc, rx = res_x[r], dry = dry: ops.conv1d_wgrad(rx, dry, Cout, 1, 1, 1, 0, outs[0], dbias = outs[1], accumulate = acc))
			res_grads += [drx, drw, drb, drg, drbeta]
		return (None, dx, dw, db, dgamma, dbeta, None, *res_grads)


class LogSoftmaxFunction(torch.autograd.Function):

	@staticmethod
	def forward(ctx, logits):
		lp = ops.log_softmax(ops.as_cl(logits, torch.float32))
		ctx.save_for_backward(lp)
		return lp

	@staticmethod
	def backward(ctx, g):
		lp, = ctx.saved_tensors
		return ops.log_softmax_bwd(g, lp)


class CtcLossFunction(torch.autograd.Function):

	@staticmethod
	def forward(ctx, log_probs, targets, olen, ylen, blank, norm = None):
		lp = ops.as_cl(log_probs, torch.float32)
		need = log_probs.requires_grad
		nll, grad = ops.ctc_loss(lp, targets, olen, ylen, blank, need_grad = need)
		ctx.norm = norm
		if need:
			ctx.save_for_backward(grad)
		if norm is None:
			return nll
		if norm.dtype == torch.int64 and norm.ndim == 1 and norm.device == nll.device:
			return ops.scale_rows(nll, None, norm)
		return nll / norm

	@staticmethod
	def backward(ctx, g):
		grad, = ctx.saved_tensors
		return ops.scale_rows(grad, g, ctx.norm), None, None, None, None, None


def ctc_loss(log_probs, targets, olen, ylen, blank, norm = None):
	return CtcLossFunction.apply(log_probs, targets, olen, ylen, blank, norm)
```

convasr_amd/ops.py:

```python
import math
import os

import ctypes

import torch

from . import _lib
from ._lib import call, ptr, stream_ptr, dtype_code, require_cuda

HALF_DTYPES = (torch.bfloat16, torch.float16)

ACT_CODES = dict(none = _lib.ACT_NONE, relu = _lib.ACT_RELU, hardtanh = _lib.ACT_HARDTANH, leaky_relu = _lib.ACT_LEAKY_RELU)


def act_args(nonlinearity):
	if nonlinearity is None:
		return _lib.ACT_NONE, 0.0, 0.0
	name = nonlinearity[0]
	if name == 'relu':
		return _lib.ACT_RELU, 0.0, 0.0
	if name == 'hardtanh':
		return _lib.ACT_HARDTANH, float(nonlinearity[1]), float(nonlinearity[2])
	if name == 'leaky_relu':
		return _lib.ACT_LEAKY_RELU, float(nonlinearity[1]) if len(nonlinearity) > 1 else 0.01, 0.0
# ... 300 lines not shown
	return dw



SPLIT_INPUT, SPLIT_GRAD = 0, 1


def split3(x, dtype, order):
	B, C, T = x.shape
	assert is_cl(x) and x.dtype == torch.float32 and dtype in HALF_DTYPES and C % 8 == 0
	out = empty_cl(B, 3 * C, T, dtype, x.device)
	_lib.timed('hbm:split3_kernel', 0.0, lambda: call('convasr_split3', ptr(x), ptr(out), dtype_code(dtype), B * T, C, int(order), stream_ptr()), nbytes = float(B * T * C * 10))
	return out


def split3_frames(x3):
	B, C3, T = x3.shape
	assert is_cl(x3) and C3 % 3 == 0
	return x3.as_strided((B, C3 // 3, 3 * T), (T * C3, 1, C3 // 3))


def split3_plane(x3, plane = 0):
	B, C3, T = x3.shape
	C = C3 // 3
	assert is_cl(x3) and C3 % 3 == 0
	out = empty_cl(B, C, T, x3.dtype, x3.device)
	out.permute(0, 2, 1).copy_(x3.as_strided((B, T, C), (T * C3, C3, 1), x3.storage_offset() + plane * C))
	return out


def conv1d_wgrad_hi(x3, dy, Cout, K, dil, pad, dw, accumulate = False, work = None, family = None):
	B, C3, Tin = x3.shape
	Cin, Tout = C3 // 3, dy.shape[2]
	layout = weight_layout(dw)
	assert is_cl(x3) and is_cl(dy) and x3.dtype == dy.dtype and x3.dtype in HALF_DTYPES and layout is not None and dw.dtype == torch.float32 and tuple(dw.shape) == (Cout, Cin, K), (dw.shape, dw.stride())
	skey = (x3.dtype, B, Cin, Cout, Tin, Tout, K, dil)
	ok = _wgrad_ld_ok.get(skey)
	if ok is None:
		ok = _wgrad_ld_ok[skey] = bool(_lib.load().convasr_conv1d_wgrad_ld_supported(dtype_code(x3.dtype), B, Cin, Cout, Tin, Tout, K, dil, C3, Cout))
	if not ok:
		return conv1d_wgrad(split3_plane(x3), dy, Cout, K, 1, dil, pad, dw, accumulate = accumulate, work = work, family = family)
	if K == 1 and (Cout * Cin) % 4 == 0:
		layout = _lib.W_KMAJOR
	wkey = (B, Cin, Cout, Tin, Tout, K, 1, dil)
	nbytes = _wgrad_ws_bytes.get(wkey)
	if nbytes is None:
		nbytes = _wgrad_ws_bytes[wkey] = _lib.load().convasr_conv1d_wgrad_workspace_bytes(*wkey)
	ws = workspace(nbytes, x3.device, 'wgrad')
	_lib.timed(family or 'conv1d_wgrad', 2.0 * B * Tout * Cout * Cin * K if work is None else work, lambda: call('convasr_conv1d_wgrad_ld', ptr(x3), C3, ptr(dy), Cout, ptr(dw), ptr(ws), dtype_code(dy.dtype), B, Cin, Cout, Tin, Tout, K, dil, pad, int(accumulate), layout, stream_ptr()))
	return dw


_wgrad_ld_ok = {}


def pack_weight_split3(w, dtype, out = None, want_dgrad = True, dgrad_planes = 3):
	require_cuda(w)
	w = w.detach()
	layout = weight_layout(w) if w.dtype == torch.float32 else None
	if layout is None:
		w, layout = w.float().contiguous(), _lib.W_REFERENCE
	Cout, Cin, K = w.shape
	fwd, dgr = out if out is not None else (None, None)
	if fwd is None:
		fwd = torch.zeros(K, cout_pad(Cout), 3 * Cin, dtype = dtype, device = w.device)
	if dgr is None and want_dgrad:
		dgr = torch.zeros(K, cout_pad(Cin), dgrad_planes * Cout, dtype = dtype, device = w.device)
	assert dgr is None or dgr.shape[2] == dgrad_planes * Cout
	call('convasr_pack_conv_weight_split3', ptr(w), layout, ptr(fwd), ptr(dgr) if want_dgrad else None, dgrad_planes, dtype_code(dtype), Cout, Cin, K, stream_ptr())
	return fwd, (dgr if want_dgrad else None)


def colsum(y, out, accumulate = False):
	B, C, T = y.shape
	assert is_cl(y) and out.dtype == torch.float32 and out.numel() == C and out.is_contiguous()
	ws = workspace(_lib.load().convasr_colsum_workspace_bytes(B * T, C), y.device, 'colsum')
	call('convasr_colsum', ptr(y), dtype_code(y.dtype), B * T, C, ptr(out), ptr(ws), int(accumulate), stream_ptr())
	return out


_wgrad_ws_bytes = {}


def conv1d_wgrad(x, dy, Cout, K, stride, dil, pad, dw, dbias = None, accumulate = False, work = None, family = None):
	B, Cin, Tin = x.shape
	Tout = dy.shape[2]
	layout = weight_layout(dw)
	assert is_cl(x) and is_cl(dy) and x.dtype == dy.dtype and layout is not None and dw.dtype == torch.float32 and tuple(dw.shape) == (Cout, Cin, K), (dw.shape, dw.stride())
	if K == 1 and (Cout * Cin) % 4 == 0:
		layout = _lib.W_KMAJOR
	wkey = (B, Cin, Cout, Tin, Tout, K, stride, dil)
	nbytes = _wgrad_ws_bytes.get(wkey)
	if nbytes is None:
		nbytes = _wgrad_ws_bytes[wkey] = _lib.load().convasr_conv1d_wgrad_workspace_bytes(*wkey)
	ws = workspace(nbytes, x.device, 'wgrad')
	_lib.timed(family or 'conv1d_wgrad', 2.0 * B * Tout * Cout * Cin * K if work is None else work, lambda: call('convasr_conv1d_wgrad', ptr(x), ptr(dy), ptr(dw), ptr(dbias), ptr(ws), dtype_code(x.dtype), B, Cin, Cout, Tin, Tout, K, stride, dil, pad, int(accumulate), layout, stream_ptr()))
	return dw



def grouped_conv1d(x, w, bias, groups, stride = 1, pad = 0, relu = True):
	B, Cin, Tin = x.shape
	Cout, cgi, K = w.shape
	assert is_cl(x) and w.dtype == torch.float32 and cgi * groups == Cin
	Tout = conv_out_len(Tin, K, stride, 1, pad)
	y = empty_cl(B, Cout, Tout, x.dtype, x.device)
	call('convasr_grouped_conv1d_fwd', ptr(x), ptr(w), w.stride(0), w.stride(1), w.stride(2), ptr(bias), ptr(y), dtype_code(x.dtype), B, Cin, Cout, Tin, Tout, K, stride, pad, groups, int(relu), stream_ptr())
	return y


def grouped_conv1d_dgrad(dy, y_act, w, Cin, Tin, groups, stride = 1, pad = 0):
	B, Cout, Tout = dy.shape
	K = w.shape[2]
	assert is_cl(dy) and (y_act is None or (is_cl(y_act) and y_act.dtype == dy.dtype))
	dx = empty_cl(B, Cin, Tin, dy.dtype, dy.device)
	call('convasr_grouped_conv1d_dgrad', ptr(dy), ptr(y_act), ptr(w), w.stride(0), w.stride(1), w.stride(2), ptr(dx), dtype_code(dy.dtype), B, Cin, Cout, Tin, Tout, K, stride, pad, groups, stream_ptr())
	return dx


def grouped_conv1d_wgrad(x, dy, y_act, dw, dbias, groups, stride = 1, pad = 0, accumulate = False):
	B, Cin, Tin = x.shape
	Cout, Tout, K = dy.shape[1], dy.shape[2], dw.shape[2]
	assert is_cl(x) and is_cl(dy) and dw.dtype == torch.float32 and tuple(dw.shape) == (Cout, Cin // groups, K)
	ws = workspace(_lib.load().convasr_grouped_conv1d_wgrad_workspace_bytes(B, Cin, Cout, K, groups), x.device, 'grouped_wgrad')
	call('convasr_grouped_conv1d_wgrad', ptr(x), ptr(dy), ptr(y_act), ptr(dw), dw.stride(0), dw.stride(1), dw.stride(2), ptr(dbias), ptr(ws), dtype_code(x.dtype), B, Cin, Cout, Tin, Tout, K, stride, pad, groups, int(accumulate), stream_ptr())
	return dw



def bn_finalize(stats, n, gamma, beta, running_mean, running_var, momentum, eps, num_batches_tracked = None):
	if isinstance(stats, ConvStats):
		buf, rows, C = stats.buf, stats.rows, stats.C
	else:
		buf, rows, C = stats, 1, stats.numel() // 2
	out = torch.empty(4, C, dtype = torch.float32, device = buf.device)
	o = out.data_ptr()
	call('convasr_bn_finalize', ptr(buf), rows, n, ptr(gamma), ptr(beta), ptr(running_mean), ptr(running_var), float(momentum), float(eps), o, o + 4 * C, o + 8 * C, o + 12 * C, C, ptr(num_batches_tracked), stream_ptr())
	return out


def _float_array(vals):
	return (ctypes.c_float * max(len(vals), 1))(*[float(v) for v in vals])


def bn_finalize_grouped(stats, n, gammas, betas, running_means, running_vars, momenta, epss, num_batches_tracked):
	k, C, rows = len(stats), stats[0].C, stats[0].rows
	assert all(s_.C == C and s_.rows == rows for s_ in stats)
	out = torch.empty(k, 4, C, dtype = torch.float32, device = stats[0].buf.device)
	call('convasr_bn_finalize_grouped', k, _ptr_array([s_.buf for s_ in stats]), rows, n, _ptr_array(gammas), _ptr_array(betas), _ptr_array(running_means), _ptr_array(running_vars),
		_float_array(momenta), _float_array(epss), _ptr_array([out[i] for i in range(k)]), _ptr_array(num_batches_tracked), C, stream_ptr())
	return [out[i] for i in range(k)]


def bn_bwd_finalize_grouped(sums, gammas, means, invstds, n, coefs, dgammas, dbetas, accumulate):
	k, C = len(sums), sums[0].numel() // 2
	call('convasr_bn_bwd_finalize_grouped', k, _ptr_array(sums), _int_array([1] * k), _ptr_array(gammas), _ptr_array(means), _ptr_array(invstds), _ptr_array(coefs), _ptr_array(dgammas), _ptr_array(dbetas),
		_int_array(accumulate), int(n), C, stream_ptr())


def bn_bwd_reduce_many(dz, gate, dropout_p, ys, means, invstds, gammas, coefs, dgammas, dbetas, accumulate):
	B, C, T = dz.shape
	assert is_cl(dz) and dz.dtype in HALF_DTYPES and all(is_cl(y) and y.dtype == dz.dtype and y.shape == dz.shape for y in ys) and gate.dtype == torch.uint8 and gate.numel() * 8 == dz.numel()
	g = empty_cl(B, C, T, dz.dtype, dz.device)
	k = len(ys)
	ws = workspace(_lib.load().convasr_bn_bwd_reduce_many_workspace_bytes(k, B, T, C), dz.device, 'bn_bwd')
	_lib.timed('hbm:bn_act_bwd_reduce_kernel', 0.0, lambda: call('convasr_bn_bwd_reduce_many', ptr(dz), ptr(gate), float(dropout_p), ptr(g), k, _ptr_array(ys), _ptr_array(means), _ptr_array(invstds), _ptr_array(gammas),
		_ptr_array(coefs), _ptr_array(dgammas), _ptr_array(dbetas), _int_array(accumulate), ptr(ws), dtype_code(dz.dtype), B, T, C, stream_ptr()), nbytes = float(B * T * C * dz.element_size() * (2 + k)))
	return g


def bn_bwd_apply_grouped(g, ys, coefs):
	B, C, T = g.shape
	assert is_cl(g) and g.dtype in HALF_DTYPES and all(is_cl(y) and y.dtype == g.dtype and y.shape == g.shape for y in ys)
	dys = [empty_cl(B, C, T, g.dtype, g.device) for _ in ys]
	_lib.timed('hbm:bn_act_bwd_apply_kernel', 0.0, lambda: call('convasr_bn_bwd_apply_grouped', ptr(g), len(ys), _ptr_array(ys), _ptr_array(coefs), _ptr_array(dys), dtype_code(g.dtype), B, T, C, stream_ptr()), nbytes = float(B * T * C * g.element_size() * (1 + 2 * len(ys))))
	return dys


def bn_eval_scale_shift(gamma, beta, running_mean, running_var, eps):
# ... 88 lines not shown
	targets = targets.to(device = dev, dtype = torch.int64).contiguous()
	if targets.ndim == 1:
		targets = targets.view(B, -1)
	olen = olen.to(device = dev, dtype = torch.int64).contiguous()
	ylen = ylen.to(device = dev, dtype = torch.int64).contiguous()
	S_max = targets.shape[1]
	nbytes = _lib.load().convasr_ctc_workspace_bytes(B, T, S_max)
	if nbytes < 0:
		raise _lib.ConvasrHipError(f'ctc_loss: target length {S_max} unsupported')
	ws = workspace(nbytes, dev, 'ctc')
	nll = torch.empty(B, dtype = torch.float32, device = dev)
	grad = empty_cl(B, C, T, torch.float32, dev) if need_grad else None
	call('convasr_ctc_loss', ptr(log_probs), ptr(targets), ptr(olen), ptr(ylen), ptr(nll), ptr(grad), ptr(ws), B, T, C, S_max, blank, stream_ptr())
	return nll, grad


def scale_rows(grad, gscale, gdiv = None):
	B = grad.shape[0]
	out = torch.empty_like(grad)
	assert gdiv is None or (gdiv.dtype == torch.int64 and gdiv.ndim == 1 and gdiv.shape[0] == B and gdiv.device == grad.device)
	call('convasr_scale_rows', ptr(grad), None if gscale is None else ptr(gscale.to(torch.float32).contiguous()), ptr(gdiv), 0 if gdiv is None else gdiv.stride(0), ptr(out), B, grad.numel() // B, stream_ptr())
	return out


def loss_head(loss_vec, ylen_col, ent = None, accumulate_iterations = 1, need_grad = True, loss_scaler = None, metric_scale = 1.0):
	require_cuda(loss_vec)
	B = loss_vec.shape[0]
	lv = loss_vec.detach().to(torch.float32).contiguous()
	assert ylen_col.dtype == torch.int64 and ylen_col.ndim == 1 and ylen_col.shape[0] == B and ylen_col.device == lv.device
	out3 = torch.empty(3, dtype = torch.float32, device = lv.device)
	gvec = torch.empty(B, dtype = torch.float32, device = lv.device) if need_grad else None
	skipped = torch.empty(1, dtype = torch.bool, device = lv.device)
	ent = None if ent is None else ent.detach().to(torch.float32).contiguous()
	call('convasr_loss_head', ptr(lv), ptr(ylen_col), ylen_col.stride(0), ptr(ent), B, float(accumulate_iterations), ptr(out3), ptr(gvec), ptr(skipped), ptr(loss_scaler), float(metric_scale), stream_ptr())
	return out3, gvec, skipped


def entropy(log_probs, olen = None, eps = 1e-9):
	B, C, T = log_probs.shape
	lp = as_cl(log_probs, torch.float32)
	ent = torch.empty(B, dtype = torch.float32, device = lp.device)
	ol = None if olen is None else olen.to(device = lp.device, dtype = torch.int64).contiguous()
	call('convasr_entropy', ptr(lp), ptr(ol), ptr(ent), B, T, C, float(eps), stream_ptr())
	return ent


def weighted_mean_entropy(log_probs, olen = None, eps = 1e-9, eps_id = -1):
	B, C, T = log_probs.shape
	lp = as_cl(log_probs, torch.float32)
	out = torch.empty(B, dtype = torch.float32, device = lp.device)
	ol = None if olen is None else olen.to(device = lp.device, dtype = torch.int64).contiguous()
	call('convasr_weighted_mean_entropy', ptr(lp), ptr(ol), ptr(out), B, T, C, int(eps_id) % C, float(eps), stream_ptr())
	return out


def normalize_signal(signal, eps = 1e-5, denom_multiplier = 1.0):
	require_cuda(signal)
	assert signal.ndim == 2
	if signal.numel() == 0:
		return signal
	signal = signal.contiguous() if signal.dtype in (torch.float32, torch.int16) else signal.float().contiguous()
	B, T = signal.shape
	absmax = torch.empty(B, dtype = torch.float32, device = signal.device)
	call('convasr_signal_absmax', ptr(signal), dtype_code(signal.dtype), B, T, ptr(absmax), stream_ptr())
	x = signal if signal.dtype == torch.float32 else signal.float()
	out = torch.empty_like(x)
	scale = ((absmax + eps) * denom_multiplier).reciprocal()
	call('convasr_scale_rows', ptr(x), ptr(scale), None, 0, ptr(out), B, T, stream_ptr())
	return out


def argmax(log_probs):
	B, C, T = log_probs.shape
	lp = as_cl(log_probs, torch.float32)
	idx = torch.empty(B, T, dtype = torch.int64, device = lp.device)
	call('convasr_argmax', ptr(lp), ptr(idx), B * T, C, stream_ptr())
	return idx



def sumsq(flat_grad, out = None, norm_out = None, norm_scale = 1.0, loss_scaler = None):
	out = out if out is not None else torch.empty(1, dtype = torch.float64, device = flat_grad.device)
	ws = workspace(_lib.load().convasr_sumsq_workspace_bytes(), flat_grad.device, 'sumsq')
	call('convasr_sumsq', ptr(flat_grad), flat_grad.numel(), ptr(out), ptr(ws), ptr(norm_out), float(norm_scale), ptr(loss_scaler), stream_ptr())
	return out


def _scaler_pair(scaler):
	if scaler is None:
		return None, None
	s_in, s_out = scaler
	assert s_in.dtype == s_out.dtype == torch.float32 and s_in.numel() == s_out.numel() == _lib.LOSS_SCALER_FLOATS and s_in.data_ptr() != s_out.data_ptr()
	return s_in, s_out


def sgd_step(p, g, buf, n, sumsq_buf, max_norm, lr, momentum, weight_decay, nesterov, first, grad_out = None, loss_gate = None, grad_scale = 1.0, p16 = None, scaler = None, lr_dev = None):
	assert loss_gate is None or (loss_gate.dtype == torch.float32 and loss_gate.numel() == 1)
	assert p16 is None or (p16.dtype in HALF_DTYPES and p16.numel() == n)
	s_in, s_out = _scaler_pair(scaler)
	call('convasr_sgd_step', ptr(p), ptr(g), ptr(buf), ptr(grad_out), n, ptr(sumsq_buf), float(max_norm), float(lr), float(momentum), float(weight_decay), int(nesterov), int(first), ptr(loss_gate), float(grad_scale), ptr(p16), _lib.BF16 if p16 is None else dtype_code(p16.dtype), ptr(s_in), ptr(s_out), ptr(lr_dev), stream_ptr())


def adamw_step(p, g, exp_avg, exp_avg_sq, n, sumsq_buf, max_norm, lr, beta1, beta2, eps, weight_decay, step_in, step_out, loss_gate = None, grad_scale = 1.0, p16 = None, scaler = None, lr_dev = None):
	assert loss_gate is None or (loss_gate.dtype == torch.float32 and loss_gate.numel() == 1)
	assert p16 is None or (p16.dtype in HALF_DTYPES and p16.numel() == n)
	assert step_in.dtype == step_out.dtype == torch.float32 and step_in.data_ptr() != step_out.data_ptr()
	s_in, s_out = _scaler_pair(scaler)
	call('convasr_adamw_step', ptr(p), ptr(g), ptr(exp_avg), ptr(exp_avg_sq), n, ptr(sumsq_buf), float(max_norm), float(lr), float(beta1), float(beta2), float(eps), float(weight_decay), ptr(step_in), ptr(step_out), ptr(loss_gate), float(grad_scale), ptr(p16), _lib.BF16 if p16 is None else dtype_code(p16.dtype), ptr(s_in), ptr(s_out), ptr(lr_dev), stream_ptr())


def conv1d_dgrad_bn_reduce(dy, packed_dgrad, Cin, K, dil, pad, bn_y, bn_scale, bn_shift, bn_mean, bn_invstd, act, dropout_p, seed, offset, xlen, bn_sums, work = None, gate = None, step_key = None):
	import ctypes
	B, Cout, Tdy = dy.shape
	T = conv_out_len(Tdy, K, 1, dil, pad)
	assert is_cl(dy) and dy.dtype in HALF_DTYPES and is_cl(bn_y) and bn_y.dtype == dy.dtype and tuple(bn_y.shape) == (B, Cin, T) and isinstance(bn_sums, ConvStats) and bn_sums.fits(Cin, B, T, dy.device), (dy.shape, bn_y.shape, Cin, T)
	rows = ctypes.c_int(0)
	dx = empty_cl(B, Cin, T, dy.dtype, dy.device)
	rc = [0]
	def run():
		rc[0] = _lib.call_rc('convasr_conv1d_dgrad_bn_reduce', ptr(dy), ptr(packed_dgrad), ptr(dx), dtype_code(dy.dtype), B, Cout, Cin, Tdy, T, K, dil, pad, ptr(bn_y), ptr(bn_scale), ptr(bn_shift), ptr(bn_mean), ptr(bn_invstd), act[0], act[1], act[2], float(dropout_p), int(seed), int(offset), step_key, ptr(xlen), ptr(bn_sums.buf), ctypes.byref(rows), ptr(gate), stream_ptr())
	family = 'conv1d_igemm_v2s_kernel<bf16>+bn_bwd' if Cout % 64 == 0 else 'conv1d_igemm (other variants)'
	flops, nbytes_ = 2.0 * B * T * Cout * Cin * K if work is None else work, float(B * Tdy * Cout * 2 + K * Cout * Cin * 2 + 2 * B * T * Cin * 2)
	symbol = 'v2s16' if family.startswith('conv1d_igemm_v2s') else None
	if family.startswith('conv1d_igemm_v2s') and memory_bound(flops, nbytes_):
		family = 'hbm:conv1d_igemm_v2s_kernel (memory-bound launches: the 38-class decoder)'
	_lib.timed(family, flops, run, nbytes = nbytes_, symbol = symbol)
	bn_sums.rows = rows.value
	return dx if rc[0] == 0 else None


def bn_bwd_finalize(sums, gamma, mean, invstd, n, coef = None, dgamma = None, dbeta = None, accumulate = False):
	buf, rows, C = (sums.buf, sums.rows, sums.C) if isinstance(sums, ConvStats) else (sums, 1, sums.numel() // 2)
	call('convasr_bn_bwd_finalize', ptr(buf), rows, ptr(gamma), ptr(mean), ptr(invstd), ptr(coef), ptr(dgamma), ptr(dbeta), int(accumulate), int(n), C, stream_ptr())



def novograd_work_table(offsets_host, device):
	item = _lib.load().convasr_novograd_item_elems()
	items, seg_first = [], [0]
	for s_, (lo, hi) in enumerate(zip(offsets_host[:-1], offsets_host[1:])):
		for b in range(lo, max(hi, lo + 1), item):
			items.append((s_, b, min(hi, b + item)))
		seg_first.append(len(items))
	return (torch.tensor(items, dtype = torch.int64, device = device), torch.tensor(seg_first, dtype = torch.int64, device = device), torch.empty(len(items), dtype = torch.float64, device = device))


def novograd_step(p, g, mom, ema_in, ema_out, g2, offsets, n, table, max_norm, lr, beta1, beta2, eps, weight_decay, dampening, first, loss_gate = None, total_norm = None, grad_scale = 1.0, p16 = None, scaler = None, lr_dev = None):
	items, seg_first, item_part = table
	assert offsets.dtype == torch.int64 and ema_in.data_ptr() != ema_out.data_ptr() and g2.dtype == torch.float64
	n_seg = offsets.numel() - 1
	s_in, s_out = _scaler_pair(scaler)
	assert p16 is None or (p16.dtype in HALF_DTYPES and p16.numel() == n)
	assert int(first) >= 0 or (ema_in.numel() == n_seg + 1 and ema_out.numel() == n_seg + 1), 'first = -1 (device-side first-step detection) needs the applied-step counter behind the EMAs'
	call('convasr_novograd_step', ptr(p), ptr(g), ptr(mom), ptr(ema_in), ptr(ema_out), ptr(g2), ptr(offsets), n_seg, n, ptr(items), items.shape[0], ptr(seg_first), ptr(item_part), float(max_norm or 0.0), float(lr), float(beta1), float(beta2), float(eps), float(weight_decay), int(bool(dampening)), int(first), ptr(loss_gate), ptr(total_norm), float(grad_scale), ptr(p16), _lib.BF16 if p16 is None else dtype_code(p16.dtype), ptr(s_in), ptr(s_out), ptr(lr_dev), stream_ptr())


def ctc_alignment(log_probs_btc, targets, input_lengths, target_lengths, blank):
	B, T, C = log_probs_btc.shape
	dev = log_probs_btc.device
	assert log_probs_btc.is_contiguous() and log_probs_btc.dtype == torch.float32
	targets = targets.to(device = dev, dtype = torch.int64).contiguous()
	il = input_lengths.to(device = dev, dtype = torch.int64).contiguous()
	tl = target_lengths.to(device = dev, dtype = torch.int64).contiguous()
	S_max = targets.shape[1]
	out = torch.empty(B, S_max, dtype = torch.int64, device = dev)
	ws = workspace(_lib.load().convasr_ctc_alignment_workspace_bytes(B, T, S_max), dev, 'ctc_alignment')
	call('convasr_ctc_alignment', ptr(log_probs_btc), ptr(targets), ptr(il), ptr(tl), ptr(out), ptr(ws), B, T, C, S_max, int(blank), stream_ptr())
	return out
# ... 307 lines not shown
```

convasr_amd/parallel.py:

```python
import os
import queue
import threading
import weakref

import torch
import torch.distributed as dist
import torch.nn as nn

from .train import FlatParameters


XGMI_LINK_GBS_PER_DIRECTION = 76.8


def predict_exposed_comm(params_numel, offsets, buckets, world, step_ms, link_gbs = XGMI_LINK_GBS_PER_DIRECTION, efficiency = 0.7, latency_us = 40.0, forward_share = 0.33, tail_share = 0.04, bytes_per_element = 4):
	total = float(sum(params_numel))
	bwd_share = 1.0 - forward_share - tail_share
	t_fwd, t_bwd_end = step_ms * forward_share, step_ms * (forward_share + bwd_share)
	rows, t_free = [], 0.0
	for b in sorted(buckets, key = lambda b: -b['lo']):
		above = sum(n for n, o in zip(params_numel, offsets) if o >= b['lo'])
		ready = t_fwd + (t_bwd_end - t_fwd) * above / total
		nbytes = (b['hi'] - b['lo']) * bytes_per_element
		t = 0.0 if world <= 1 else 2.0 * (nbytes / world) / (efficiency * link_gbs * 1e9) * 1e3 + latency_us * 1e-3
		start = max(ready, t_free)
		t_free = start + t
		rows.append(dict(mib = round(nbytes / 2 ** 20, 1), ready_ms = round(ready, 3), start_ms = round(start, 3), comm_ms = round(t, 3), end_ms = round(t_free, 3)))
	return dict(exposed_comm_ms = round(max(0.0, t_free - t_bwd_end), 3), comm_ms_total = round(sum(r['comm_ms'] for r in rows), 3), backward_end_ms = round(t_bwd_end, 3), step_ms = round(step_ms, 3),
		world = world, link_gbs_per_direction = link_gbs, efficiency = efficiency, latency_us = latency_us, bytes_per_element = bytes_per_element, per_bucket = rows,
		predicted_scaling = None if world <= 1 else round(world * step_ms / (step_ms + max(0.0, t_free - t_bwd_end)), 3),
		model = 'direct reduce-scatter + all-gather over one xGMI link per peer; bucket ready times from the backward pass apportioned by parameter counts; serial collectives on the communication stream (convasr_amd.parallel.predict_exposed_comm)')


class DataParallelEngine(nn.Module):
	def __init__(self, module, device = None, bucket_bytes = int(os.environ.get('CONVASR_BUCKET_MIB', 64)) << 20, process_group = None, flat = None, force_collectives = False, first_bucket_bytes = 4 << 20, fold_mean = True, comm_thread = os.environ.get('CONVASR_COMM_THREAD', '0') == '1', measure_exposed_comm = False, grad_comm_dtype = os.environ.get('CONVASR_GRAD_COMM', 'auto')):
		super().__init__()
		self.module = module
		self.group = process_group
		self.world_size = dist.get_world_size(process_group) if dist.is_initialized() else 1
		self.collectives = self.world_size > 1 or (force_collectives and dist.is_initialized())
		self.flat = flat if flat is not None else getattr(module, '_convasr_flat', None) or FlatParameters(module)
		module._convasr_flat = self.flat
		self.buckets = self._make_buckets(bucket_bytes, min(first_bucket_bytes, bucket_bytes))
		self._pending = []
		self._ready = []
		self._jobs = queue.Queue() if (comm_thread and self.collectives and self.flat.data.is_cuda) else None
		self._worker = None
		self._comm_dirty = False
		self._remaining = [len(b['params']) for b in self.buckets]
		self._main_stream = None
		self._comm_stream = None
		self.fold_mean = fold_mean
		self.sync = True
		self.grad_comm_dtype = {None: None, 'f32': None, 'auto': 'auto', 'f16': torch.float16, 'bf16': torch.bfloat16}.get(grad_comm_dtype, grad_comm_dtype)
		self._comm_bufs = {}
		self._mean_in_comm = False
		self._capture_comm = None
		for bi, b in enumerate(self.buckets):
			for p in b['params']:
				p._convasr_ready = self._make_hook(bi)
		self.measure_exposed_comm = measure_exposed_comm
		self.exposed_comm_events = []
		from . import functional as Fn
		ref, key = weakref.ref(self), id(self)
		def hook():
			eng = ref()
			if eng is None:
				Fn.after_long_launch_hooks.pop(key, None)
			else:
				eng.poll()
		Fn.after_long_launch_hooks[key] = hook
		self._hook_key = key
		if self.collectives:
			dist.broadcast(self.flat.data, src = 0, group = self.group)
			for buf in module.buffers():
				dist.broadcast(buf, src = 0, group = self.group)
			from . import functional as Fn
			Fn.bump_param_epoch()

	def close(self):
		from . import functional as Fn
		Fn.after_long_launch_hooks.pop(getattr(self, '_hook_key', None), None)
		worker, self._worker = getattr(self, '_worker', None), None
		if worker is not None and self._jobs is not None:
			self._jobs.put(None)
			worker.join(timeout = 5)

	def destroy_capture_comm(self):
		comm, self._capture_comm = self._capture_comm, None
		if comm is not None:
			comm.destroy()

	def __del__(self):
		try:
			self.close()
		except Exception:
			pass

	def predict(self, world, step_ms, **kw):
		kw.setdefault('bytes_per_element', 2 if self.comm_dtype() is not None else 4)
		return predict_exposed_comm([p.numel() for p in self.flat.params], self.flat.offsets, self.buckets, world, step_ms, **kw)

	def exposed_comm_ms(self):
		ms = [a.elapsed_time(b) for a, b in self.exposed_comm_events]
		return sum(ms) / len(ms) if ms else None

	def _make_buckets(self, bucket_bytes, first_bucket_bytes):
		flat = self.flat
		buckets, cur = [], None
		for p, off in zip(flat.params, flat.offsets):
			end = off + p.numel()
			limit = min(bucket_bytes, first_bucket_bytes << max(len(buckets) - 1, 0))
			if cur is None or (end - cur['lo']) * 4 > limit and cur['params']:
				cur = dict(lo = off, hi = end, params = [])
				buckets.append(cur)
			cur['params'].append(p)
			cur['hi'] = end
		return buckets

	def _make_hook(self, bi):
		def ready(param):
			if not self.sync:
				return
			self._remaining[bi] -= 1
			if self._remaining[bi] == 0:
				self._mark_ready(bi)
		return ready

	def _comm(self, dev):
		if self._comm_stream is None:
			self._comm_stream = torch.cuda.Stream(device = dev)
		return self._comm_stream

	def _mark_ready(self, bi):
		if not self.collectives:
			return
		view = self.flat.grad[self.buckets[bi]['lo']:self.buckets[bi]['hi']]
		if not view.is_cuda:
			self._launch(bi, ())
			return
		from . import functional as Fn
		dev = view.device
		producers = {s.cuda_stream: s for s in (self._main_stream, torch.cuda.current_stream(dev), Fn.side_stream(dev)) if s is not None}
# ... 194 lines not shown
```

convasr_amd/train.py:

```python
import math
import os

import torch

from . import ops, _lib
from . import models as M
from . import functional as Fn


class FlatParameters:
	ALIGN = 64

	def __init__(self, model):
		params = [p for p in model.parameters() if p.requires_grad]
		if not params:
			raise ValueError('model has no trainable parameters')
		dev = params[0].device
		self.params, self.offsets = params, []
		off = 0
		for p in params:
			if p.dtype != torch.float32 or p.device != dev:
				raise ValueError('FlatParameters needs fp32 parameters on one device')
			self.offsets.append(off)
			off += (p.numel() + self.ALIGN - 1) // self.ALIGN * self.ALIGN
		self.numel = off
		self.data = torch.zeros(off, dtype = torch.float32, device = dev)
		self.grad = torch.zeros(off, dtype = torch.float32, device = dev)
		self.data16 = None
		self._mirror_ver = {}
		self._as_param = []
		for p, o in zip(params, self.offsets):
			n = p.numel()
			kmajor = p.ndim == 3 and p.shape[2] > 1 and (p.shape[0] * p.shape[1]) % 8 == 0 and dev.type == 'cuda'
			as_param = (lambda flat, p = p, o = o, n = n: flat[o:o + n].view(p.shape[2], p.shape[0], p.shape[1]).permute(1, 2, 0)) if kmajor else (lambda flat, p = p, o = o, n = n: flat[o:o + n].view(p.shape))
			self._as_param.append(as_param)
			view = as_param(self.data)
			view.copy_(p.data)
			p.data = view
			p._convasr_grad = as_param(self.grad)
			p._convasr_fresh = True
			one_tap = p.ndim == 3 and p.shape[2] == 1 and (p.shape[0] * p.shape[1]) % 8 == 0 and dev.type == 'cuda'
			p._convasr_arena = (self, o) if (kmajor or one_tap) else None
			p.grad = p._convasr_grad
		self._by_id = {id(p): p for p in params}
		self.clip = None
		self.grad_scale = 1.0
		self._sumsq = torch.zeros(1, dtype = torch.float64, device = dev)
		self.loss_scaler = None

	def mirror(self, dtype = torch.bfloat16):
		if self.data16 is None or self.data16.dtype != dtype:
			assert dtype in ops.HALF_DTYPES
			self.data16 = torch.zeros(self.numel, dtype = dtype, device = self.data.device)
			self._mirror_ver = {}
		return self.data16

	def mirror_carried_over(self, run):
		was = {k for k, v in self._mirror_ver.items() if v == Fn.param_version(self._by_id[k])} if self._mirror_ver else set()
		run(self.data16)
		Fn.bump_param_epoch()
		self._mirror_ver = {k: Fn.param_version(self._by_id[k]) for k in was} if self.data16 is not None else {}

	def param_views(self, flat_tensor):
		assert flat_tensor.numel() == self.numel
		return [f(flat_tensor) for f in self._as_param]

	def export_state(self, flat_tensor):
		return [v.contiguous().clone() for v in self.param_views(flat_tensor)]

	def import_state(self, flat_tensor, per_param, what):
		if isinstance(per_param, torch.Tensor):
			raise ValueError(f'{what}: a flat arena-ordered tensor (optimizer state written before format 2) carries no layout tag and cannot be loaded safely: conv segments may be tap-major or reference-ordered')
		views = self.param_views(flat_tensor)
		if len(per_param) != len(views):
			raise ValueError(f'{what}: {len(per_param)} tensors for {len(views)} parameters')
		for v, t in zip(views, per_param):
			if tuple(v.shape) != tuple(t.shape):
				raise ValueError(f'{what}: shape {tuple(t.shape)} does not match parameter shape {tuple(v.shape)}')
			v.copy_(t)

	def zero_grad(self):
		for p in self.params:
			p._convasr_fresh = True
			p.grad = p._convasr_grad
		self.clip = None

	def grads_written_externally(self):
		for p in self.params:
			if getattr(p, '_convasr_grad_is_zero', False):
				p._convasr_grad_is_zero = False

	def finalize_grads(self):
		for p in self.params:
			if p._convasr_fresh:
				p._convasr_grad.zero_()

	def clip_grad_norm_(self, max_norm):
		self.finalize_grads()
		norm = torch.empty(1, dtype = torch.float32, device = self.grad.device)
		ops.sumsq(self.grad, self._sumsq, norm_out = norm, norm_scale = self.grad_scale, loss_scaler = None if self.loss_scaler is None else self.loss_scaler.current)
		self.clip = (self._sumsq, float(max_norm))
		return norm[0]


class LossScaler:

	def __init__(self, device, loss_scale = 'dynamic', init_scale = 2.0 ** 16, scale_factor = 2.0, scale_window = 2000, min_loss_scale = None, max_loss_scale = 2.0 ** 24):
		dynamic = loss_scale in (None, 'dynamic')
		state = [float(init_scale) if dynamic else float(loss_scale), 0.0, 0.0, float(scale_window) if dynamic else 0.0, float(min_loss_scale or 0.0), float(max_loss_scale), float(scale_factor), 0.0]
		assert len(state) == _lib.LOSS_SCALER_FLOATS
		self.state = torch.tensor([state, state], dtype = torch.float32, device = device)
		self.cur = 0
		self.pinned = False

	@property
	def current(self):
		return self.state[self.cur]

	def pair(self):
		return self.state[self.cur], self.state[1 - self.cur]

	def advance(self):
		if Fn.capturing() or self.pinned:
			_lib.call('convasr_copy', _lib.ptr(self.state[1 - self.cur]), _lib.ptr(self.state[self.cur]), 4 * _lib.LOSS_SCALER_FLOATS, _lib.stream_ptr())
		else:
			self.cur = 1 - self.cur

	def loss_scale(self):
		return float(self.current[0])

	def state_dict(self):
		s = self.current.tolist()
		return dict(loss_scale = s[0], unskipped = int(s[1]))

	def load_state_dict(self, sd):
		cur = self.current.clone()
		cur[0], cur[1] = float(sd['loss_scale']), float(sd['unskipped'])
		self.state[self.cur].copy_(cur)


def amp_state_dict(optimizer):
	scaler = getattr(getattr(optimizer, 'flat', None), 'loss_scaler', None)
	return {} if scaler is None else dict(loss_scaler0 = scaler.state_dict())


def amp_load_state_dict(optimizer, sd):
	scaler = getattr(getattr(optimizer, 'flat', None), 'loss_scaler', None)
	if scaler is not None and sd and 'loss_scaler0' in sd:
		scaler.load_state_dict(sd['loss_scaler0'])


class SGD:

	def __init__(self, flat: FlatParameters, lr = 1e-2, momentum = 0.9, weight_decay = 1e-3, nesterov = False, keep_clipped_grads = False):
		self.flat = flat
		self.param_groups = [dict(params = flat.params, lr = lr, momentum = momentum, weight_decay = weight_decay, nesterov = nesterov)]
		self.momentum_buffer = torch.zeros_like(flat.data) if momentum != 0 else None
		self.steps = 0
		self.keep_clipped_grads = keep_clipped_grads
		self.lr_dev = None

	def zero_grad(self, set_to_none = False):
		self.flat.zero_grad()

	def step(self, loss_gate = None):
		g = self.param_groups[0]
		flat = self.flat
		if flat.clip is None:
			flat.finalize_grads()
		sumsq, max_norm = flat.clip if flat.clip is not None else (None, 0.0)
		first, grad_scale = self.steps == 0, flat.grad_scale
		if first and Fn.capturing():
			raise _lib.ConvasrHipError('SGD: the first step (which initialises the momentum buffer) cannot be the one captured into a step graph')
		scaler = flat.loss_scaler
		if scaler is not None and sumsq is None:
			sumsq = ops.sumsq(flat.grad, flat._sumsq)
		flat.mirror_carried_over(lambda p16: ops.sgd_step(flat.data, flat.grad, self.momentum_buffer, flat.numel, sumsq, max_norm, g['lr'], g['momentum'], g['weight_decay'], g['nesterov'], first, grad_out = flat.grad if self.keep_clipped_grads else None, loss_gate = loss_gate, grad_scale = grad_scale, p16 = p16, scaler = None if scaler is None else scaler.pair(), lr_dev = self.lr_dev if Fn.capturing() else None))
		if scaler is not None:
			scaler.advance()
		if self.keep_clipped_grads:
			flat.grads_written_externally()
		self.steps += 1
		flat.clip, flat.grad_scale = None, 1.0
# ... 306 lines not shown
```

include/convasr_hip.h:

```cpp
#ifndef CONVASR_HIP_H
#define CONVASR_HIP_H

#include <stdint.h>

#ifdef __cplusplus
extern "C" {
#endif

#define CONVASR_ABI_VERSION 10

enum { CONVASR_F32 = 0, CONVASR_BF16 = 1, CONVASR_I16 = 2, CONVASR_F16 = 3 };
enum { CONVASR_ACT_NONE = 0, CONVASR_ACT_RELU = 1, CONVASR_ACT_HARDTANH = 2, CONVASR_ACT_LEAKY_RELU = 3 };
enum { CONVASR_OK = 0, CONVASR_EINVAL = -1, CONVASR_ELAUNCH = -2, CONVASR_EUNSUPPORTED = -3 };

int convasr_abi_version(void);
const char* convasr_last_error(void);


int convasr_convert_layout(const void* src, int src_dtype, int64_t src_sb, int64_t src_sc, int64_t src_st,
                           void* dst, int dst_dtype, int64_t dst_sb, int64_t dst_sc, int64_t dst_st,
                           int B, int C, int T, void* stream);


int convasr_signal_absmax(const void* signal, int signal_dtype, int B, int T, float* absmax, void* stream);

int convasr_logmel_fwd(const void* signal, int signal_dtype, const float* absmax, const float* xlen,
                       const float* window, int win_length, const float* mel_weight, const float* mel_bias,
                       float* out, int B, int T, int nfft, int hop, int nmel, float preemphasis, void* stream);


int convasr_instnorm_fwd(const void* x, int x_dtype, int64_t x_sb, int64_t x_sc, int64_t x_st,
                         void* y, int y_dtype, int64_t y_sb, int64_t y_sc, int64_t y_st,
                         const float* xlen, int B, int C, int T, int T_out, float eps, void* stream);

int convasr_instnorm_running_fwd(const void* x, int x_dtype, int64_t x_sb, int64_t x_sc, int64_t x_st,
                                 void* y, int y_dtype, int64_t y_sb, int64_t y_sc, int64_t y_st,
                                 int B, int C, int T, int T_out, float eps, float* running_mean, float* running_var,
                                 int64_t* num_batches_tracked, float momentum, int training, float* stats_workspace, void* stream);


int convasr_output_lengths(const float* xlen, int B, int T, int64_t* out, void* stream);


int convasr_conv_cout_pad(int cout);

#define CONVASR_W_REFERENCE 0
#define CONVASR_W_KMAJOR 1

int convasr_pack_conv_weight(const float* w, void* packed_fwd, void* packed_dgrad, int dtype, int Cout, int Cin, int K, int w_layout, void* stream);

int convasr_conv1d_fwd(const void* x, const void* wp, void* y, int x_dtype, int y_dtype,
                       int B, int Cin, int Cout, int Tin, int Tout, int K, int stride, int dil, int pad,
                       const float* bias, double* stats, const float* scale, const float* shift,
                       int act, float act_lo, float act_hi, const float* xlen, int* stats_rows, void* stream);
int convasr_conv_stats_max_rows(int B, int Tout);

int convasr_conv1d_fwd_splitk_plan(int x_dtype, int B, int Cin, int Cout, int Tout, int K, int64_t* workspace_bytes);
int convasr_conv1d_fwd_splitk(const void* x, const void* wp, void* y, int x_dtype, int y_dtype,
                              int B, int Cin, int Cout, int Tin, int Tout, int K, int dil, int pad,
                              const float* bias, const float* scale, const float* shift, int act, float act_lo, float act_hi,
                              const float* xlen, int splits, void* workspace, void* stream);

int convasr_fold2_geometry(int K, int pad, int* K_folded, int* pad_folded);
int convasr_fold2_pack_weight(const float* w, int w_layout, void* packed_fwd, int dtype, int Cout, int Cin, int K, int pad, void* stream);
int convasr_fold2_unfold_wgrad(const float* dw_folded, float* dw, int dw_layout, int Cout, int Cin, int K, int pad, int accumulate, void* stream);

int convasr_debug_set_conv_v2(int enable);

int64_t convasr_conv1d_wgrad_workspace_bytes(int B, int Cin, int Cout, int Tin, int Tout, int K, int stride, int dil);

int convasr_conv1d_wgrad(const void* x, const void* dy, float* dw, float* dbias, void* workspace, int dtype,
                         int B, int Cin, int Cout, int Tin, int Tout, int K, int stride, int dil, int pad,
                         int accumulate, int dw_layout, void* stream);


int convasr_grouped_conv1d_fwd(const void* x, const float* w, int64_t w_sco, int64_t w_sj, int64_t w_sk, const float* bias, void* y, int dtype,
                               int B, int Cin, int Cout, int Tin, int Tout, int K, int stride, int pad, int groups, int relu, void* stream);
int convasr_grouped_conv1d_dgrad(const void* dy, const void* y_act, const float* w, int64_t w_sco, int64_t w_sj, int64_t w_sk, void* dx, int dtype,
                                 int B, int Cin, int Cout, int Tin, int Tout, int K, int stride, int pad, int groups, void* stream);
int64_t convasr_grouped_conv1d_wgrad_workspace_bytes(int B, int Cin, int Cout, int K, int groups);
int convasr_grouped_conv1d_wgrad(const void* x, const void* dy, const void* y_act, float* dw, int64_t w_sco, int64_t w_sj, int64_t w_sk, float* dbias,
                                 void* workspace, int dtype, int B, int Cin, int Cout, int Tin, int Tout, int K, int stride, int pad, int groups,
                                 int accumulate, void* stream);


int convasr_bn_finalize(const double* stats, int stats_rows, int64_t n, const float* gamma, const float* beta,
                        float* running_mean, float* running_var, float momentum, float eps,
                        float* mean, float* invstd, float* scale, float* shift, int C,
                        int64_t* num_batches_tracked, void* stream);
int convasr_reduce_rows(const double* part, int rows, int width, double* out, void* stream);

int convasr_bn_eval_scale_shift(const float* gamma, const float* beta, const float* running_mean, const float* running_var,
                                float eps, float* scale, float* shift, int C, void* stream);

int convasr_bn_act_fwd(const void* y, void* z, int dtype, const float* scale, const float* shift,
                       int n_res, const void* const* res, const float* const* rscale, const float* const* rshift,
                       int act, float act_lo, float act_hi, float dropout_p, uint64_t seed, uint64_t offset, const uint64_t* step_key,
                       const float* xlen, int B, int T, int C, uint8_t* gate, void* stream);

int64_t convasr_bn_bwd_workspace_bytes(int B, int T, int C);
int convasr_bn_act_bwd_reduce(const void* dz, const void* y, void* g, int dtype, const float* scale, const float* shift,
                              const float* mean, const float* invstd,
                              int n_res, const void* const* res, const float* const* rscale, const float* const* rshift,
                              const float* const* rmean, const float* const* rinvstd, double* const* rsums,
                              int act, float act_lo, float act_hi, float dropout_p, uint64_t seed, uint64_t offset, const uint64_t* step_key,
                              const float* xlen, double* sums, void* workspace, const float* gamma, float* coef, float* dgamma, float* dbeta,
                              int accumulate, int B, int T, int C, const uint8_t* gate, void* stream);

int convasr_bn_act_bwd_apply(const void* dz_or_g, const void* y, void* dy, int dtype, const float* coef, int from_dz,
                             const float* scale, const float* shift, int act, float act_lo, float act_hi, float dropout_p,
                             uint64_t seed, uint64_t offset, const uint64_t* step_key, const float* xlen, int B, int T, int C, const uint8_t* gate, void* stream);

int convasr_bn_bwd_apply(const void* g, const void* y, void* dy, int dtype, const float* gamma, const float* mean,
                         const float* invstd, const double* sums, float* dgamma, float* dbeta, int accumulate,
                         int B, int T, int C, void* stream);


int convasr_log_softmax_fwd(const float* logits, float* log_probs, int64_t rows, int C, void* stream);
int convasr_log_softmax_bwd(const float* grad_lp, const float* log_probs, float* dlogits, int64_t rows, int C, void* stream);

int64_t convasr_ctc_workspace_bytes(int B, int T, int S_max);
int convasr_ctc_loss(const float* log_probs, const int64_t* targets, const int64_t* olen, const int64_t* ylen,
                     float* nll, float* grad, void* workspace, int B, int T, int C, int S_max, int blank, void* stream);
int convasr_scale_rows(const float* grad, const float* gscale, const int64_t* gdiv, int64_t gdiv_stride, float* out, int B, int64_t per_b, void* stream);

int convasr_loss_head(const float* loss_vec, const int64_t* ylen, int64_t ylen_stride, const float* entropy, int B, float accumulate_iterations, float* out3,
                      float* grad_loss_vec, unsigned char* skipped, const float* loss_scaler, float metric_scale, void* stream);

#define CONVASR_LOSS_SCALER_FLOATS 8

int convasr_entropy(const float* log_probs, const int64_t* olen, float* ent, int B, int T, int C, float eps, void* stream);
int convasr_weighted_mean_entropy(const float* log_probs, const int64_t* olen, float* out, int B, int T, int C, int eps_id, float eps, void* stream);
int convasr_argmax(const float* log_probs, int64_t* idx, int64_t rows, int C, void* stream);


int64_t convasr_sumsq_workspace_bytes(void);
int convasr_sumsq(const float* g, int64_t n, double* sumsq, void* workspace, float* norm_out, float norm_scale, const float* loss_scaler, void* stream);
int convasr_sgd_step(float* p, const float* g, float* buf, float* grad_out, int64_t n, const double* sumsq, float max_norm,
                     float lr, float momentum, float weight_decay, int nesterov, int first, const float* loss_gate, float grad_scale,
                     void* p16, int p16_dtype, const float* scaler_in, float* scaler_out, const float* lr_dev, void* stream);
int convasr_adamw_step(float* p, const float* g, float* exp_avg, float* exp_avg_sq, int64_t n, const double* sumsq, float max_norm, float lr,
                       float beta1, float beta2, float eps, float weight_decay, const float* step_in, float* step_out, const float* loss_gate,
                       float grad_scale, void* p16, int p16_dtype, const float* scaler_in, float* scaler_out, const float* lr_dev, void* stream);

int convasr_conv1d_dgrad_bn_reduce(const void* dy, const void* packed_dgrad, void* dx, int dtype, int B, int Cout, int Cin, int T_dy, int T_dx, int K,
                                   int dil, int pad, const void* bn_y, const float* bn_scale, const float* bn_shift, const float* bn_mean,
                                   const float* bn_invstd, int bn_act, float bn_act_lo, float bn_act_hi, float dropout_p, uint64_t seed,
                                   uint64_t offset, const uint64_t* step_key, const float* bn_xlen, double* bn_sums, int* bn_rows, const uint8_t* bn_gate, void* stream);
int convasr_bn_bwd_finalize(const double* sums, int sums_rows, const float* gamma, const float* mean, const float* invstd, float* coef,
                            float* dgamma, float* dbeta, int accumulate, int64_t n, int C, void* stream);


int convasr_conv1x1_grouped(int n, const void* const* x, const void* const* w, void* const* y, const float* const* bias, double* const* stats,
                            const int* cin, const int* cout, const int* accumulate, int dtype, int B, int T, int* stats_rows, void* stream);
int64_t convasr_wgrad1x1_grouped_workspace_bytes(int n, const int* cin, const int* cout, int B, int T);
int convasr_wgrad1x1_grouped(int n, const void* const* x, const void* const* dy, float* const* dw, float* const* zero, const int* cin, const int* cout,
                             const int* accumulate, void* workspace, int dtype, int B, int T, void* stream);
int convasr_bn_finalize_grouped(int count, const double* const* stats, int stats_rows, int64_t n, const float* const* gamma, const float* const* beta,
                                float* const* running_mean, float* const* running_var, const float* momentum, const float* eps, float* const* out,
                                int64_t* const* num_batches_tracked, int C, void* stream);
int convasr_bn_bwd_finalize_grouped(int count, const double* const* sums, const int* sums_rows, const float* const* gamma, const float* const* mean,
                                    const float* const* invstd, float* const* coef, float* const* dgamma, float* const* dbeta, const int* accumulate,
                                    int64_t n, int C, void* stream);
int convasr_bn_bwd_apply_grouped(const void* g, int count, const void* const* y, const float* const* coef, void* const* dy, int dtype, int B, int T, int C, void* stream);
int64_t convasr_bn_bwd_reduce_many_workspace_bytes(int count, int B, int T, int C);
int convasr_bn_bwd_reduce_many(const void* dz, const uint8_t* gate, float dropout_p, void* g, int count, const void* const* y, const float* const* mean,
                               const float* const* invstd, const float* const* gamma, float* const* coef, float* const* dgamma, float* const* dbeta,
                               const int* accumulate, void* workspace, int dtype, int B, int T, int C, void* stream);
int convasr_add16(const void* a, const void* b, void* out, int64_t n, int dtype, void* stream);

int convasr_pack_dgrad_item_bytes(void);
int convasr_pack_dgrad_grouped(const void* items, int n_items, int total_blocks, void* stream);

int64_t convasr_colsum_workspace_bytes(int64_t rows, int C);
int convasr_colsum(const void* y, int dtype, int64_t rows, int C, float* out, void* workspace, int accumulate, void* stream);

int convasr_cast_scale(const void* src, int src_dtype, void* dst, int dst_dtype, int64_t n, float scale, void* stream);


int convasr_split3(const float* x, void* out, int dtype, int64_t rows, int C, int order, void* stream);
int convasr_bn_act_fwd_split3(const void* y, void* z3, int plane_dtype, const float* scale, const float* shift,
                              int n_res, const void* const* res, const float* const* rscale, const float* const* rshift,
                              int act, float act_lo, float act_hi, float dropout_p, uint64_t seed, uint64_t offset, const uint64_t* step_key,
                              const float* xlen, int B, int T, int C, uint8_t* gate, void* stream);
int convasr_bn_act_bwd_apply_split3(const void* dz_or_g, const void* y, void* dy3, int plane_dtype, const float* coef, int from_dz,
                                    const float* scale, const float* shift, int act, float act_lo, float act_hi, float dropout_p,
                                    uint64_t seed, uint64_t offset, const uint64_t* step_key, const float* xlen, int B, int T, int C,
                                    const uint8_t* gate, void* stream);
int convasr_pack_conv_weight_split3(const float* w, int w_layout, void* packed_fwd, void* packed_dgrad, int dgrad_planes, int dtype, int Cout, int Cin, int K, void* stream);
int convasr_bn_act_bwd_apply_to_half(const void* dz_or_g, const void* y, void* dy16, int out_dtype, const float* coef, int from_dz,
                                     const float* scale, const float* shift, int act, float act_lo, float act_hi, float dropout_p,
                                     uint64_t seed, uint64_t offset, const uint64_t* step_key, const float* xlen, int B, int T, int C,
                                     const uint8_t* gate, void* stream);
int convasr_conv1d_wgrad_ld_supported(int dtype, int B, int Cin, int Cout, int Tin, int Tout, int K, int dil, int x_ld, int dy_ld);
int convasr_conv1d_wgrad_ld(const void* x, int x_ld, const void* dy, int dy_ld, float* dw, void* workspace, int dtype,
                            int B, int Cin, int Cout, int Tin, int Tout, int K, int dil, int pad, int accumulate, int dw_layout, void* stream);


int convasr_step_begin(uint64_t* state, void* stream);
int convasr_copy(const void* src, void* dst, int64_t nbytes, void* stream);


int convasr_novograd_step(float* p, const float* g, float* mom, const float* ema_in, float* ema_out, double* g2, const int64_t* offsets,
                          int n_seg, int64_t n, const int64_t* items, int n_items, const int64_t* seg_first, double* item_part,
                          float max_norm, float lr, float beta1, float beta2, float eps, float weight_decay, int dampening, int first,
                          const float* loss_gate, float* total_norm, float grad_scale, void* p16, int p16_dtype, const float* scaler_in,
                          float* scaler_out, const float* lr_dev, void* stream);
int64_t convasr_novograd_item_elems(void);

int64_t convasr_ctc_alignment_workspace_bytes(int B, int T, int S_max);
int convasr_ctc_alignment(const float* log_probs, const int64_t* targets, const int64_t* input_lengths, const int64_t* target_lengths,
                          int64_t* alignment, void* workspace, int B, int T, int C, int S_max, int blank, void* stream);

int convasr_ctc_alignment_long_states_per_block(void);
int convasr_ctc_alignment_long_chunk_frames(void);
int64_t convasr_ctc_alignment_long_workspace_bytes(int B, int T, int S_max);
int convasr_ctc_alignment_long(const float* log_probs, const int64_t* targets, const int64_t* input_lengths, const int64_t* target_lengths,
                               int64_t* alignment, void* workspace, int64_t workspace_bytes, int B, int T, int C, int S_max, int blank,
                               int chunk_frames, void* stream);
int convasr_ctc_alignment_long_parts(const float* log_probs, const int64_t* targets, const int64_t* input_lengths, const int64_t* target_lengths,
// ... 86 lines not shown
```

Baseline: 59410.

## Fuse gradient sum-of-squares into K-major wgrad combine for norm clipping

The K-major wgrad reduction kernel now optionally computes per-block partial sums of squares of the final weight gradient while writing it. The arena builds a plan of these slots plus fixed-size chunks for parameters not covered, so clip_grad_norm only reduces the uncovered chunks and the partials instead of re-reading the whole flat gradient. This removes a full pass over the gradient arena at the cost of extra double-precision work in the combine kernel and state tracking for whether every fused slot was refreshed. It is disabled under gradient exchange, and the plan is built only after a first step with the old path.

```diff
diff --git a/convasr_amd/_lib.py b/convasr_amd/_lib.py
--- a/convasr_amd/_lib.py
+++ b/convasr_amd/_lib.py
@@ -58,6 +58,11 @@
 	convasr_argmax = (c_int, [c_p, c_p, c_i64, c_int, c_p]),
 	convasr_sumsq_workspace_bytes = (c_i64, []),
 	convasr_sumsq = (c_int, [c_p, c_i64, c_p, c_p, c_p, c_f32, c_p, c_p]),
+	convasr_sumsq_chunk = (c_int, []),
+	convasr_sumsq_fused = (c_int, [c_p, c_p, c_int, c_p, c_int, c_p, c_p, c_f32, c_p, c_p]),
+	convasr_wgrad_sumsq_parts = (c_i64, [c_i64]),
+	convasr_conv1d_wgrad_sumsq = (c_int, [c_p, c_p, c_p, c_p, c_p, c_int, c_int, c_int, c_int, c_int, c_int, c_int, c_int, c_int, c_int, c_int, c_p, c_p]),
+	convasr_wgrad_combine_kmajor = (c_int, [c_p, c_p, c_int, c_i64, c_int, c_p, c_p]),
 	convasr_sgd_step = (c_int, [c_p, c_p, c_p, c_p, c_i64, c_p, c_f32, c_f32, c_f32, c_f32, c_int, c_int, c_p, c_f32, c_p, c_int, c_p, c_p, c_p, c_p]),
 	convasr_adamw_step = (c_int, [c_p, c_p, c_p, c_p, c_i64, c_p, c_f32, c_f32, c_f32, c_f32, c_f32, c_f32, c_p, c_p, c_p, c_f32, c_p, c_int, c_p, c_p, c_p, c_p]),
 	convasr_conv1d_dgrad_bn_reduce = (c_int, [c_p, c_p, c_p, c_int, c_int, c_int, c_int, c_int, c_int, c_int, c_int, c_int, c_p, c_p, c_p, c_p, c_p, c_int, c_f32, c_f32, c_f32, c_u64, c_u64, c_p, c_p, c_p, c_p, c_p, c_p]),
diff --git a/convasr_amd/csrc/conv.hip b/convasr_amd/csrc/conv.hip
--- a/convasr_amd/csrc/conv.hip
+++ b/convasr_amd/csrc/conv.hip
@@ -745,16 +745,33 @@
 	}
 }
 
-__global__ __launch_bounds__(256) void wgrad_reduce_kmajor_kernel(const float* __restrict__ slab, float* __restrict__ dw, int S, int64_t n4, int accumulate) {
+template <bool NORM>
+__global__ __launch_bounds__(256) void wgrad_reduce_kmajor_kernel(const float* __restrict__ slab, float* __restrict__ dw, int S, int64_t n4, int accumulate, double* __restrict__ sumsq_part) {
 	const float4* const s4 = reinterpret_cast<const float4*>(slab);
 	float4* const d4 = reinterpret_cast<float4*>(dw);
+	double sq = 0.0;
 	for (int64_t i = (int64_t)blockIdx.x * 256 + threadIdx.x; i < n4; i += (int64_t)gridDim.x * 256) {
 		float4 a = s4[i];
 		for (int s = 1; s < S; ++s) { const float4 b = s4[(int64_t)s * n4 + i]; a.x += b.x; a.y += b.y; a.z += b.z; a.w += b.w; }
 		if (accumulate) { const float4 o = d4[i]; a.x += o.x; a.y += o.y; a.z += o.z; a.w += o.w; }
 		d4[i] = a;
-	}
-}
+		if constexpr (NORM) sq += (double)a.x * (double)a.x + (double)a.y * (double)a.y + (double)a.z * (double)a.z + (double)a.w * (double)a.w;
+	}
+	if constexpr (NORM) {
+		__shared__ double red[4];
+#pragma unroll
+		for (int o = 32; o > 0; o >>= 1) sq += __shfl_xor(sq, o, 64);
+		if ((threadIdx.x & 63) == 0) red[threadIdx.x >> 6] = sq;
+		__syncthreads();
+		if (threadIdx.x == 0) sumsq_part[blockIdx.x] = ((red[0] + red[1]) + red[2]) + red[3];
+	}
+}
+
+static int64_t wgrad_reduce_kmajor_blocks(int64_t n4) {
+	const int64_t blocks = ceil_div64(n4, 256);
+	return blocks > 2048 ? 2048 : blocks;
+}
+extern "C" int64_t convasr_wgrad_sumsq_parts(int64_t n) { return n > 0 && (n & 3) == 0 ? wgrad_reduce_kmajor_blocks(n >> 2) : -1; }
 
 template <typename T> __global__ __launch_bounds__(256) void colsum_kernel(const T* __restrict__ y, float* __restrict__ part, int64_t rows, int C, int rows_per_block) {
 	__shared__ float red[4][64];
@@ -835,7 +852,8 @@
 }
 
 static int wgrad_impl(const void* x, int x_ld, const void* dy, int dy_ld, float* dw, float* dbias, void* workspace, int dtype, int B, int Cin, int Cout, int Tin,
-                      int Tout, int K, int stride, int dil, int pad, int accumulate, int dw_layout, void* stream) {
+                      int Tout, int K, int stride, int dil, int pad, int accumulate, int dw_layout, void* stream, double* sumsq_part = nullptr) {
+	CONVASR_CHECK_ARG(!sumsq_part || dw_layout == CONVASR_W_KMAJOR, "conv1d_wgrad_sumsq: only the K-major combine forms the partial sums of squares");
 	CONVASR_CHECK_ARG(x && dy && dw && workspace && B > 0 && Cin > 0 && Cout > 0 && Tin > 0 && Tout > 0 && K > 0 && stride > 0 && dil > 0 && (dw_layout == CONVASR_W_REFERENCE || dw_layout == CONVASR_W_KMAJOR), "conv1d_wgrad: bad arguments");
 	CONVASR_CHECK_ARG(dw_layout == CONVASR_W_REFERENCE || (((int64_t)Cout * Cin) & 3) == 0, "conv1d_wgrad: K-major dw needs Cout * Cin %% 4 == 0");
 	CONVASR_CHECK_ARG(K <= 64, "conv1d_wgrad: K %d > 64", K);
@@ -856,9 +874,9 @@
 	CONVASR_CHECK_LAUNCH("conv1d_wgrad");
 	if (dw_layout == CONVASR_W_KMAJOR) {
 		const int64_t n4 = (int64_t)K * Cout * Cin / 4;
-		int64_t blocks = ceil_div64(n4, 256);
-		if (blocks > 2048) blocks = 2048;
-		hipLaunchKernelGGL(wgrad_reduce_kmajor_kernel, dim3((unsigned)blocks), dim3(256), 0, s, (const float*)p.slab, dw, p.splits, n4, accumulate);
+		const int64_t blocks = wgrad_reduce_kmajor_blocks(n4);
+		if (sumsq_part) hipLaunchKernelGGL(wgrad_reduce_kmajor_kernel<true>, dim3((unsigned)blocks), dim3(256), 0, s, (const float*)p.slab, dw, p.splits, n4, accumulate, sumsq_part);
+		else hipLaunchKernelGGL(wgrad_reduce_kmajor_kernel<false>, dim3((unsigned)blocks), dim3(256), 0, s, (const float*)p.slab, dw, p.splits, n4, accumulate, (double*)nullptr);
 	} else hipLaunchKernelGGL(wgrad_reduce_kernel, dim3((Cin + 63) / 64, Cout), dim3(256), (size_t)K * 65 * sizeof(float), s, p.slab, dw, p.splits, K, Cout, Cin, accumulate);
 	CONVASR_CHECK_LAUNCH("conv1d_wgrad_reduce");
 	if (dbias) {
@@ -880,6 +898,21 @@
 	return wgrad_impl(x, 0, dy, 0, dw, dbias, workspace, dtype, B, Cin, Cout, Tin, Tout, K, stride, dil, pad, accumulate, dw_layout, stream);
 }
 
+extern "C" int convasr_conv1d_wgrad_sumsq(const void* x, const void* dy, float* dw, float* dbias, void* workspace, int dtype, int B, int Cin, int Cout, int Tin,
+                                          int Tout, int K, int stride, int dil, int pad, int accumulate, double* sumsq_part, void* stream) {
+	CONVASR_CHECK_ARG(sumsq_part, "conv1d_wgrad_sumsq: sumsq_part is NULL");
+	return wgrad_impl(x, 0, dy, 0, dw, dbias, workspace, dtype, B, Cin, Cout, Tin, Tout, K, stride, dil, pad, accumulate, CONVASR_W_KMAJOR, stream, sumsq_part);
+}
+
+extern "C" int convasr_wgrad_combine_kmajor(const float* slab, float* dw, int S, int64_t n, int accumulate, double* sumsq_part, void* stream) {
+	CONVASR_CHECK_ARG(slab && dw && S > 0 && n > 0 && (n & 3) == 0 && (((uintptr_t)slab | (uintptr_t)dw) & 15) == 0, "wgrad_combine_kmajor: n %% 4 == 0, 16-byte aligned operands");
+	const int64_t n4 = n >> 2, blocks = wgrad_reduce_kmajor_blocks(n4);
+	if (sumsq_part) hipLaunchKernelGGL(wgrad_reduce_kmajor_kernel<true>, dim3((unsigned)blocks), dim3(256), 0, (hipStream_t)stream, slab, dw, S, n4, accumulate, sumsq_part);
+	else hipLaunchKernelGGL(wgrad_reduce_kmajor_kernel<false>, dim3((unsigned)blocks), dim3(256), 0, (hipStream_t)stream, slab, dw, S, n4, accumulate, (double*)nullptr);
+	CONVASR_CHECK_LAUNCH("wgrad_combine_kmajor");
+	return 0;
+}
+
 extern "C" int convasr_conv1d_wgrad_ld(const void* x, int x_ld, const void* dy, int dy_ld, float* dw, void* workspace, int dtype, int B, int Cin, int Cout, int Tin,
                                        int Tout, int K, int dil, int pad, int accumulate, int dw_layout, void* stream) {
 	CONVASR_CHECK_ARG(x_ld >= Cin && dy_ld >= Cout && (x_ld & 7) == 0 && (dy_ld & 7) == 0 && convasr_is_half(dtype), "conv1d_wgrad_ld: x_ld >= Cin, dy_ld >= Cout, multiples of 8, 16-bit storage");
diff --git a/convasr_amd/csrc/misc.hip b/convasr_amd/csrc/misc.hip
--- a/convasr_amd/csrc/misc.hip
+++ b/convasr_amd/csrc/misc.hip
@@ -445,6 +445,29 @@
 	return 0;
 }
 
+#define SUMSQ_CHUNK 4096
+__global__ __launch_bounds__(256) void sumsq_chunks_kernel(const float* __restrict__ g, const int64_t* __restrict__ chunks, double* __restrict__ part) {
+	__shared__ double red[4];
+	const int64_t start = chunks[2 * blockIdx.x], len = chunks[2 * blockIdx.x + 1];
+	double acc = 0.0;
+	for (int64_t j = threadIdx.x; j < len; j += 256) { const double v = (double)g[start + j]; acc += v * v; }
+#pragma unroll
+	for (int o = 32; o > 0; o >>= 1) acc += __shfl_xor(acc, o, 64);
+	if ((threadIdx.x & 63) == 0) red[threadIdx.x >> 6] = acc;
+	__syncthreads();
+	if (threadIdx.x == 0) part[blockIdx.x] = ((red[0] + red[1]) + red[2]) + red[3];
+}
+
+extern "C" int convasr_sumsq_chunk(void) { return SUMSQ_CHUNK; }
+
+extern "C" int convasr_sumsq_fused(const float* g, const int64_t* chunks, int n_chunks, double* parts, int n_parts, double* sumsq, float* norm_out, float norm_scale, const float* loss_scaler, void* stream) {
+	CONVASR_CHECK_ARG(g && parts && sumsq && n_chunks >= 0 && n_parts > 0 && n_chunks <= n_parts && (n_chunks == 0 || chunks), "sumsq_fused: bad arguments");
+	if (n_chunks) hipLaunchKernelGGL(sumsq_chunks_kernel, dim3((unsigned)n_chunks), dim3(256), 0, (hipStream_t)stream, g, chunks, parts + (n_parts - n_chunks));
+	hipLaunchKernelGGL(sumsq_final_kernel, dim3(1), dim3(256), 0, (hipStream_t)stream, (const double*)parts, n_parts, sumsq, norm_out, norm_scale, loss_scaler);
+	CONVASR_CHECK_LAUNCH("sumsq_fused");
+	return 0;
+}
+
 template <typename H> __global__ __launch_bounds__(256) void sgd_step_kernel(float* __restrict__ p, const float* __restrict__ g, float* __restrict__ buf, float* __restrict__ gout,
                                                        int64_t n, const double* __restrict__ sumsq, float max_norm, float lr, float mom, float wd, int nesterov, int first,
                                                        const float* __restrict__ loss_gate, float grad_scale, H* __restrict__ p16, const float* __restrict__ scaler_in, float* __restrict__ scaler_out, const float* __restrict__ lr_dev) {
diff --git a/convasr_amd/functional.py b/convasr_amd/functional.py
--- a/convasr_amd/functional.py
+++ b/convasr_amd/functional.py
@@ -121,6 +121,16 @@
 _prepack_streams = {}
 
 
+FUSED_TAIL = os.environ.get('CONVASR_NO_FUSED_TAIL') != '1'
+
+
+def _norm_slots(weight, out):
+	arena = getattr(weight, '_convasr_arena', None)
+	if arena is None or out is None or out is not getattr(weight, '_convasr_grad', None):
+		return None
+	return arena[0].norm_slots(weight)
+
+
 GROUPED_PACK_MIN = int(os.environ.get('CONVASR_GROUPED_PACK_MIN', 32))
 _pack_tables = {}
 
@@ -272,6 +282,9 @@
 		fresh = {bool(getattr(p, '_convasr_fresh', True)) for p, ok in zip(params, live) if ok}
 		if len(fresh) != 1:
 			raise _lib.ConvasrHipError('gradient arenas of one layer are out of step (mixed fresh / accumulated state)')
+		for p, ok in zip(params, live):
+			if ok:
+				p._convasr_norm_ok = False
 		compute(arenas, not fresh.pop())
 		for p, ok in zip(params, live):
 			if ok:
@@ -295,6 +308,9 @@
 			if len(fresh) != 1:
 				raise _lib.ConvasrHipError('gradient arenas of one layer are out of step (mixed fresh / accumulated state)')
 			outs.append(arenas); accs.append(not fresh.pop()); ret.append([None] * len(params)); arena_groups.append((params, live))
+			for p, ok in zip(params, live):
+				if ok:
+					p._convasr_norm_ok = False
 		else:
 			o = [torch.empty_like(p, dtype = torch.float32, memory_format = torch.contiguous_format) if ok else None for p, ok in zip(params, live)]
 			outs.append(o); accs.append(False); ret.append(o)
@@ -721,7 +737,7 @@
 			xv = x.as_strided((Bx, 2 * Cin, Tin // 2), (Tin * Cin, 1, 2 * Cin))
 			wg = lambda: _deliver([weight], lambda outs, acc: Fold2.wgrad(xv, dy, weight, spec, ctx.fold[0], ctx.fold[1], outs[0], acc))
 		else:
-			wg = lambda: _deliver([weight], lambda outs, acc: ops.conv1d_wgrad(x, dy, Cout, spec.K, spec.stride, spec.dilation, spec.padding, outs[0], accumulate = acc))
+			wg = lambda: _deliver([weight], lambda outs, acc: ops.conv1d_wgrad(x, dy, Cout, spec.K, spec.stride, spec.dilation, spec.padding, outs[0], accumulate = acc, sumsq_part = _norm_slots(weight, outs[0])))
 		after = WGRAD_AFTER_DGRAD and arena_mode and _side_streams.get(dev) is not None
 		if arena_mode and not after:
 			dw, = _run_wgrad(dev, (x, dy), wg)
@@ -973,7 +989,7 @@
 			if spec.stride != 1:
 				raise _lib.ConvasrHipError('conv1d dgrad with stride > 1 is not implemented')
 			dx = _dgrad(x, dy, weight, spec, dt, ctx.producer_link)
-		dw, db = _deliver([weight, bias], lambda outs, acc: ops.conv1d_wgrad(x, dy, Cout, spec.K, spec.stride, spec.dilation, spec.padding, outs[0], dbias = outs[1], accumulate = acc))
+		dw, db = _deliver([weight, bias], lambda outs, acc: ops.conv1d_wgrad(x, dy, Cout, spec.K, spec.stride, spec.dilation, spec.padding, outs[0], dbias = outs[1], accumulate = acc, sumsq_part = _norm_slots(weight, outs[0])))
 		return None, dx, dw, db
 
 
@@ -1115,7 +1131,7 @@
 		else:
 			g = ops.bn_act_bwd_reduce(dz, y, scale, shift, None, None, act, write_g = True, **common)
 		dy = g if scale is None else ops.bn_act_bwd_apply(g, y, ConvBnActFrozenStatsFunction._coef(scale, Cout, dev), False)
-		dw, db = _deliver([weight, bias], lambda outs, acc: ops.conv1d_wgrad(x, dy, Cout, spec.K, spec.stride, spec.dilation, spec.padding, outs[0], dbias = outs[1], accumulate = acc))
+		dw, db = _deliver([weight, bias], lambda outs, acc: ops.conv1d_wgrad(x, dy, Cout, spec.K, spec.stride, spec.dilation, spec.padding, outs[0], dbias = outs[1], accumulate = acc, sumsq_part = _norm_slots(weight, outs[0])))
 		dx = None
 		if ctx.x_needs_grad:
 			if spec.stride != 1:
diff --git a/convasr_amd/ops.py b/convasr_amd/ops.py
--- a/convasr_amd/ops.py
+++ b/convasr_amd/ops.py
@@ -406,7 +406,7 @@
 _wgrad_ws_bytes = {}
 
 
-def conv1d_wgrad(x, dy, Cout, K, stride, dil, pad, dw, dbias = None, accumulate = False, work = None, family = None):
+def conv1d_wgrad(x, dy, Cout, K, stride, dil, pad, dw, dbias = None, accumulate = False, work = None, family = None, sumsq_part = None):
 	B, Cin, Tin = x.shape
 	Tout = dy.shape[2]
 	layout = weight_layout(dw)
@@ -418,7 +418,19 @@
 	if nbytes is None:
 		nbytes = _wgrad_ws_bytes[wkey] = _lib.load().convasr_conv1d_wgrad_workspace_bytes(*wkey)
 	ws = workspace(nbytes, x.device, 'wgrad')
+	if sumsq_part is not None:
+		assert layout == _lib.W_KMAJOR and sumsq_part.dtype == torch.float64 and sumsq_part.numel() == _lib.load().convasr_wgrad_sumsq_parts(dw.numel())
+		_lib.timed(family or 'conv1d_wgrad', 2.0 * B * Tout * Cout * Cin * K if work is None else work, lambda: call('convasr_conv1d_wgrad_sumsq', ptr(x), ptr(dy), ptr(dw), ptr(dbias), ptr(ws), dtype_code(x.dtype), B, Cin, Cout, Tin, Tout, K, stride, dil, pad, int(accumulate), ptr(sumsq_part), stream_ptr()))
+		return dw
 	_lib.timed(family or 'conv1d_wgrad', 2.0 * B * Tout * Cout * Cin * K if work is None else work, lambda: call('convasr_conv1d_wgrad', ptr(x), ptr(dy), ptr(dw), ptr(dbias), ptr(ws), dtype_code(x.dtype), B, Cin, Cout, Tin, Tout, K, stride, dil, pad, int(accumulate), layout, stream_ptr()))
+	return dw
+
+
+def wgrad_combine_kmajor(slabs, dw, accumulate = False, sumsq_part = None):
+	S, n = slabs.shape
+	assert slabs.dtype == dw.dtype == torch.float32 and slabs.is_contiguous() and dw.is_contiguous() and dw.numel() == n
+	assert sumsq_part is None or (sumsq_part.dtype == torch.float64 and sumsq_part.numel() == _lib.load().convasr_wgrad_sumsq_parts(n))
+	call('convasr_wgrad_combine_kmajor', ptr(slabs), ptr(dw), S, n, int(accumulate), ptr(sumsq_part), stream_ptr())
 	return dw
 
 
@@ -673,8 +685,46 @@
 def sumsq(flat_grad, out = None, norm_out = None, norm_scale = 1.0, loss_scaler = None):
 	out = out if out is not None else torch.empty(1, dtype = torch.float64, device = flat_grad.device)
 	ws = workspace(_lib.load().convasr_sumsq_workspace_bytes(), flat_grad.device, 'sumsq')
-	call('convasr_sumsq', ptr(flat_grad), flat_grad.numel(), ptr(out), ptr(ws), ptr(norm_out), float(norm_scale), ptr(loss_scaler), stream_ptr())
-	return out
+	_lib.timed('sumsq', 0.0, lambda: call('convasr_sumsq', ptr(flat_grad), flat_grad.numel(), ptr(out), ptr(ws), ptr(norm_out), float(norm_scale), ptr(loss_scaler), stream_ptr()), nbytes = 4.0 * flat_grad.numel(), symbol = 'sumsq_kernel')
+	return out
+
+
+class ArenaNorm:
+
+	def __init__(self, numel, fused, device):
+		lib = _lib.load()
+		chunk = lib.convasr_sumsq_chunk()
+		self.numel, self.fused = int(numel), [(int(o), int(n)) for o, n in fused]
+		self.slot_of, chunks, pos, nslots = [], [], 0, 0
+		order = sorted(range(len(self.fused)), key = lambda i: self.fused[i][0])
+		bases = {}
+		for i in order:
+			o, n = self.fused[i]
+			if o < pos or n <= 0 or n % 4 or o % 4 or o + n > self.numel:
+				raise ValueError(f'ArenaNorm: range ({o}, {n}) overlaps its predecessor, leaves the arena or is not 4-element aligned')
+			chunks += [(s, min(chunk, o - s)) for s in range(pos, o, chunk)]
+			bases[i] = (nslots, int(lib.convasr_wgrad_sumsq_parts(n)))
+			nslots += bases[i][1]
+			pos = o + n
+		chunks += [(s, min(chunk, self.numel - s)) for s in range(pos, self.numel, chunk)]
+		self.slot_of = [bases[i] for i in range(len(self.fused))]
+		self.chunks = chunks
+		self.n_parts = nslots + len(chunks)
+		self.parts = torch.zeros(max(self.n_parts, 1), dtype = torch.float64, device = device)
+		self.table = torch.tensor(chunks, dtype = torch.int64).reshape(-1, 2).to(device) if chunks else None
+
+	def slots(self, i):
+		base, n = self.slot_of[i]
+		return self.parts[base:base + n]
+
+	def ranges(self):
+		return list(self.fused), list(self.chunks)
+
+	def finish(self, flat_grad, out = None, norm_out = None, norm_scale = 1.0, loss_scaler = None):
+		assert flat_grad.numel() == self.numel and flat_grad.dtype == torch.float32 and flat_grad.device == self.parts.device and self.n_parts > 0
+		out = out if out is not None else torch.empty(1, dtype = torch.float64, device = flat_grad.device)
+		_lib.timed('sumsq', 0.0, lambda: call('convasr_sumsq_fused', ptr(flat_grad), ptr(self.table), len(self.chunks), ptr(self.parts), self.n_parts, ptr(out), ptr(norm_out), float(norm_scale), ptr(loss_scaler), stream_ptr()), nbytes = 8.0 * self.n_parts, symbol = 'sumsq_chunks_kernel')
+		return out
 
 
 def _scaler_pair(scaler):
diff --git a/convasr_amd/parallel.py b/convasr_amd/parallel.py
--- a/convasr_amd/parallel.py
+++ b/convasr_amd/parallel.py
@@ -59,6 +59,8 @@
 		for bi, b in enumerate(self.buckets):
 			for p in b['params']:
 				p._convasr_ready = self._make_hook(bi)
+		if self.collectives:
+			self.flat.grad_exchange = True
 		self.measure_exposed_comm = measure_exposed_comm
 		self.exposed_comm_events = []
 		from . import functional as Fn
diff --git a/convasr_amd/train.py b/convasr_amd/train.py
--- a/convasr_amd/train.py
+++ b/convasr_amd/train.py
@@ -47,6 +47,8 @@
 		self.grad_scale = 1.0
 		self._sumsq = torch.zeros(1, dtype = torch.float64, device = dev)
 		self.loss_scaler = None
+		self.grad_exchange = False
+		self._norm_plan, self._norm_params, self._norm_candidates = None, [], {}
 
 	def mirror(self, dtype = torch.bfloat16):
 		if self.data16 is None or self.data16.dtype != dtype:
@@ -79,7 +81,29 @@
 				raise ValueError(f'{what}: shape {tuple(t.shape)} does not match parameter shape {tuple(v.shape)}')
 			v.copy_(t)
 
+	def norm_slots(self, p):
+		if self.grad_exchange or not Fn.FUSED_TAIL or p.numel() % 4:
+			return None
+		if self._norm_plan is None:
+			self._norm_candidates[id(p)] = p
+			return None
+		i = self._norm_index.get(id(p))
+		if i is None:
+			return None
+		p._convasr_norm_ok = True
+		return self._norm_plan.slots(i)
+
+	def _plan_norm(self):
+		off = {id(p): o for p, o in zip(self.params, self.offsets)}
+		self._norm_params = [p for p in self._norm_candidates.values() if id(p) in off and p._convasr_grad.data_ptr() == self.grad.data_ptr() + 4 * off[id(p)]]
+		self._norm_candidates = {}
+		if self._norm_params:
+			self._norm_plan = ops.ArenaNorm(self.numel, [(off[id(p)], p.numel()) for p in self._norm_params], self.grad.device)
+			self._norm_index = {id(p): i for i, p in enumerate(self._norm_params)}
+
 	def zero_grad(self):
+		for p in self._norm_params:
+			p._convasr_norm_ok = False
 		for p in self.params:
 			p._convasr_fresh = True
 			p.grad = p._convasr_grad
@@ -89,6 +113,8 @@
 		for p in self.params:
 			if getattr(p, '_convasr_grad_is_zero', False):
 				p._convasr_grad_is_zero = False
+		for p in self._norm_params:
+			p._convasr_norm_ok = False
 
 	def finalize_grads(self):
 		for p in self.params:
@@ -98,7 +124,13 @@
 	def clip_grad_norm_(self, max_norm):
 		self.finalize_grads()
 		norm = torch.empty(1, dtype = torch.float32, device = self.grad.device)
-		ops.sumsq(self.grad, self._sumsq, norm_out = norm, norm_scale = self.grad_scale, loss_scaler = None if self.loss_scaler is None else self.loss_scaler.current)
+		scaler = None if self.loss_scaler is None else self.loss_scaler.current
+		if self._norm_plan is not None and not self.grad_exchange and all(getattr(p, '_convasr_norm_ok', False) for p in self._norm_params):
+			self._norm_plan.finish(self.grad, self._sumsq, norm_out = norm, norm_scale = self.grad_scale, loss_scaler = scaler)
+		else:
+			ops.sumsq(self.grad, self._sumsq, norm_out = norm, norm_scale = self.grad_scale, loss_scaler = scaler)
+			if self._norm_plan is None and self._norm_candidates and not Fn.capturing():
+				self._plan_norm()
 		self.clip = (self._sumsq, float(max_norm))
 		return norm[0]
 
diff --git a/include/convasr_hip.h b/include/convasr_hip.h
--- a/include/convasr_hip.h
+++ b/include/convasr_hip.h
@@ -72,6 +72,12 @@
 int convasr_conv1d_wgrad(const void* x, const void* dy, float* dw, float* dbias, void* workspace, int dtype,
                          int B, int Cin, int Cout, int Tin, int Tout, int K, int stride, int dil, int pad,
                          int accumulate, int dw_layout, void* stream);
+
+int64_t convasr_wgrad_sumsq_parts(int64_t n);
+int convasr_conv1d_wgrad_sumsq(const void* x, const void* dy, float* dw, float* dbias, void* workspace, int dtype,
+                               int B, int Cin, int Cout, int Tin, int Tout, int K, int stride, int dil, int pad,
+                               int accumulate, double* sumsq_part, void* stream);
+int convasr_wgrad_combine_kmajor(const float* slab, float* dw, int S, int64_t n, int accumulate, double* sumsq_part, void* stream);
 
 
 int convasr_grouped_conv1d_fwd(const void* x, const float* w, int64_t w_sco, int64_t w_sj, int64_t w_sk, const float* bias, void* y, int dtype,
@@ -136,6 +142,9 @@
 
 int64_t convasr_sumsq_workspace_bytes(void);
 int convasr_sumsq(const float* g, int64_t n, double* sumsq, void* workspace, float* norm_out, float norm_scale, const float* loss_scaler, void* stream);
+int convasr_sumsq_chunk(void);
+int convasr_sumsq_fused(const float* g, const int64_t* chunks, int n_chunks, double* parts, int n_parts, double* sumsq, float* norm_out,
+                        float norm_scale, const float* loss_scaler, void* stream);
 int convasr_sgd_step(float* p, const float* g, float* buf, float* grad_out, int64_t n, const double* sumsq, float max_norm,
                      float lr, float momentum, float weight_decay, int nesterov, int first, const float* loss_gate, float grad_scale,
                      void* p16, int p16_dtype, const float* scaler_in, float* scaler_out, const float* lr_dev, void* stream);
```

Result: no change. 59190 (-0.4%).
